# zhvng/open-musiclm

Hardware: AMD Instinct MI355X
Metric: train steps/sec + AR tokens/sec, coarse-stage musiclm_small (higher is better)
Workload: dtype fp16ff; 1 GPU; musiclm_small coarse-stage train step (fwd+bwd+allreduce+clip+AdamW), N=1116 (3 start + 13 clap + 200 semantic + 900 coarse), forgetful mask 0.15, ff_dropout 0.1; global_batch=32, per_gpu_batch=32, grad_accum=1, seq_len=1116, parallelism=dp1, precision=fp16ff, hip_graph=True, exchange=none (single GPU)

## Files before the change

### include/omlm.h

```cpp
#ifndef OMLM_H
#define OMLM_H
#include <stdint.h>
#ifdef __cplusplus
extern "C" {
#endif

int         omlm_version(void);
const char* omlm_last_error(void);
void        omlm_set_error(const char* msg);

int omlm_gemm(const void* A, const void* B, void* C, const float* Cin,
              const int* a_map, const int* b_map, const int* c_map, long long a_rows, long long b_rows,
              int M, int N, int K, int lda, int ldb, int ldc, int ldcin,
              int a_kmajor, int b_kmajor, int in_dtype, int out_dtype, float alpha,
              void* workspace, long long workspace_bytes, void* stream);
long long omlm_gemm_tail_workspace_bytes(int M, int N);

int omlm_layernorm_fwd(const float* x, const float* gamma, void* y, void* xcast, float* mean, float* rstd,
                       int M, int D, int ldy, float eps, int out_dtype, void* stream);
int omlm_layernorm_fwd_planes(const float* x, const float* gamma, void* y, void* y_lo, float* mean, float* rstd,
                              int M, int D, int ldy, float eps, int out_dtype, void* stream);
long long omlm_layernorm_bwd_workspace_bytes(int D);
int omlm_layernorm_bwd2(const void* dy, const float* x, const float* gamma, const float* mean, const float* rstd,
                        const float* dres, const void* dres2, float* dx, void* dxcast, float* dgamma, float* workspace, int M, int D,
                        float dx_scale, int cast_dtype, int dy_dtype, void* stream);

int omlm_qk_norm_fwd(const float* q_raw, const float* kv_raw, const float* q_scale, const float* k_scale,
                     void* q, void* k, void* v, int M, int H, int out_dtype, void* stream);
int omlm_qk_norm_bwd(const float* dq, const float* dk, const float* dv, const float* q_raw, const float* kv_raw,
                     const float* q_scale, const float* k_scale, void* dq_raw, void* dkv_raw,
                     float* dq_scale, float* dk_scale, int M, int H, int out_dtype, void* stream);

int omlm_gemm_qknorm(const void* A, const void* B, void* C, void* C2, int c2_col0, int ldc2, const float* scale, float* norm_out,
                     int ldnorm, int groups, long long a_rows, long long b_rows, int M, int N, int K, int lda, int ldb, int ldc,
                     int dtype, void* stream);
int omlm_qk_norm_bwd2(const float* dq, const float* dk, const float* dv, const void* q, const void* k, const float* qn, const float* kn,
                      const float* q_scale, const float* k_scale, void* dq_raw, void* dkv_raw, float* dq_scale, float* dk_scale,
                      int M, int H, int dtype, void* stream);

int omlm_mqa_attn_fwd(const void* q, const void* k, const void* v, const float* bias, const float* biasT, const unsigned char* keymask,
                      void* out, float* lse, int B, int N, int H, float scale, int bias_ld, int dtype, int P, float p,
                      unsigned long long seed, const unsigned long long* seed_dev, void* stream);
long long omlm_attn_bias_table_floats(int N, int H, int P);
int omlm_attn_bias_prepare(const float* bias, float* biasT, int N, int H, int bias_ld, const float* q_scale,
                           const float* k_scale, float qk_bound, float scale, int p_max_log2, void* stream);
int omlm_attn_bias_prepare_group(const float* bias, float* const* biasT, int layers, int N, int H, int bias_ld,
                                 const float* const* q_scale, const float* const* k_scale, float qk_bound, float scale,
                                 int p_max_log2, int P, void* stream);
long long omlm_mqa_attn_bwd_workspace_bytes(int B, int N, int H);
int omlm_mqa_attn_bwd(const void* q, const void* k, const void* v, const float* bias, const float* biasT, const unsigned char* keymask,
                      const void* out, const void* dout, const float* lse, float* delta, float* dq, float* dk, float* dv, float* dbias,
                      float* dbias_ws, int B, int N, int H, float scale, int bias_ld, int dtype, int P, float p, unsigned long long seed,
                      const unsigned long long* seed_dev, void* stream);
int omlm_attn_dropout_keep(unsigned char* keep, int B, int N, int H, float p, unsigned long long seed,
                           const unsigned long long* seed_dev, void* stream);
int omlm_dropout_residual_fwd(const float* x, const float* y, float* x1, long long M, int D, float p, unsigned long long seed,
                              const unsigned long long* seed_dev, void* stream);
int omlm_dropout_residual_bwd(const float* dx1, void* dy, long long M, int D, float p, unsigned long long seed,
                              const unsigned long long* seed_dev, int out_dtype, void* stream);

int omlm_ffmid_fwd(const void* h1, const void* convw, const void* gamma, void* h2, float* mean, float* rstd,
                   int M, int nseq, int F, int Fp, float eps, float p, unsigned long long seed,
                   const unsigned long long* seed_dev, unsigned char* drop_bits, void* gh, int dtype, void* stream);
int omlm_ffmid_fwd_planes(const void* h1, const void* h1_lo, const void* convw, const void* convw_lo, const void* gamma, const void* gamma_lo,
                          void* h2, void* h2_lo, float* mean, float* rstd, int M, int nseq, int F, int Fp, float eps, float p,
                          unsigned long long seed, const unsigned long long* seed_dev, unsigned char* drop_bits, void* gh, int dtype, void* stream);
long long omlm_ffmid_bwd_workspace_bytes(int F, int Fp);
int omlm_ffmid_bwd(const void* dh2, const void* h1, const void* convw, const void* gamma, const float* mean,
                   const float* rstd, void* du_tmp, void* dh1, float* dgamma, float* dconv, float* workspace,
                   int M, int nseq, int F, int Fp, float p, unsigned long long seed,
                   const unsigned long long* seed_dev, const unsigned char* drop_bits, const void* gh, int dtype, void* stream);
int omlm_colsum_accumulate(const float* part, float* out, int P, int C, int ldp, void* stream);
typedef struct omlm_colsum_desc { const float* part; float* out; int P, C, ldp; } omlm_colsum_desc;
int omlm_colsum_group(const omlm_colsum_desc* problems, int count, void* stream);
int omlm_ffmid_set_impl(int impl);

int omlm_embed_gather_fwd(const int* ids, const int* seg, const int* posidx,
                          const float* const* tables, const float* const* starts, const float* const* pos,
                          int nseq, float* out, int B, int N, int D,
                          const long long* table_rows, const long long* pos_rows, int* err_flag, void* stream);
int omlm_embed_gather_bwd(const int* ids, const int* seg, const int* posidx,
                          float* const* dtables, float* const* dstarts, float* const* dpos,
                          int nseq, const float* dx, int B, int N, int D, float alpha,
                          const long long* table_rows, const long long* pos_rows, int* err_flag, void* stream);

int omlm_prepare_train_batch(const long long* const* ids, int* const* labels, const int* len, const int* eos, const int* Q,
                             const int* codebook, int nseq, int B, int pad_id, const float* scores, int n_drop,
                             int* ids32, unsigned char* keymask, int N, void* stream);

int omlm_cross_entropy_fwd(const float* logits, const int* labels, float* row_lse, float* nll_sum,
                           int R, int V, int ld, int* err_flag, void* stream);
int omlm_cross_entropy_bwd(const float* logits, const int* labels, const float* row_lse, const float* gscale,
                           float coef, void* dlogits, int R, int V, int ld, int ldd, int out_dtype, void* stream);

int omlm_sumsq_accumulate(const float* g, long long n, float* out, float* partials, void* stream);
int omlm_adamw_clip_step(float* p, float* g, float* m, float* v, void* p16, long long n,
                         float lr, float beta1, float beta2, float eps, float wd, int step,
                         float gscale, const float* gnorm_sq, float max_norm, int decoupled, int zero_grad, int p16_dtype,
                         const float* ls_state, void* stream);
int omlm_loss_scale_update(float* ls_state, const float* gnorm_sq, float growth, float backoff, int interval,
                           float scale_min, float scale_max, void* stream);

int omlm_cast_pad(const float* src, void* dst, long long R, int C, int ld_src, int ld_dst, int out_dtype, void* stream);
typedef struct omlm_cast_pad_desc { const float* src; void* dst; int R, C, ld_src, ld_dst, transpose, lo; } omlm_cast_pad_desc;
int omlm_cast_pad_group(const omlm_cast_pad_desc* problems, int count, int out_dtype, void* stream);

int omlm_gemm_planes(const void* A, long long a_plane_bytes, const void* B, long long b_plane_bytes, void* C, const float* Cin,
                     const int* a_map, const int* b_map, const int* c_map, long long a_rows, long long b_rows,
                     int M, int N, int K, int lda, int ldb, int ldc, int ldcin,
                     int a_kmajor, int b_kmajor, int out_dtype, float alpha, void* workspace, long long workspace_bytes, void* stream);
int omlm_split_planes(const float* x, void* planes, long long n, long long plane_elems, void* stream);
int omlm_gemm_planes16(const void* A, const void* A_lo, const void* B, const void* B_lo, void* C, void* C_lo, const float* Cin,
                       const int* a_map, const int* c_map, long long a_rows, long long b_rows, int M, int N, int K,
                       int lda, int ldb, int ldc, int ldcin, int dtype, void* workspace, long long workspace_bytes, void* stream);
int omlm_gemm_mx16(const void* A, const void* A8, long long a8_stride, const unsigned char* a_scale,
                   const void* B, const void* B8, long long b8_stride, const unsigned char* b_scale,
                   void* C, void* C_lo, int c_lo_bf8, const float* Cin, long long a_rows, long long b_rows,
                   int M, int N, int K, int lda, int ldb, int ldc, int ldcin,
                   void* workspace, long long workspace_bytes, void* stream);
long long omlm_gemm_mx16_workspace_bytes(int M, int N, int K);
int omlm_layernorm_fwd_mx(const float* x, const float* gamma, void* y, void* y8, long long y8_stride, unsigned char* scale8,
                          float* mean, float* rstd, int M, int D, int ldy, float eps, void* stream);
int omlm_ffmid_fwd_mx(const void* h1, const void* h1_lo, const void* convw, const void* convw_lo, const void* gamma, const void* gamma_lo,
                      void* h2, void* h2_8, long long h2_8_stride, unsigned char* scale8, float* mean, float* rstd, int M, int nseq, int F, int Fp,
                      float eps, float p, unsigned long long seed, const unsigned long long* seed_dev, unsigned char* drop_bits, void* gh, void* stream);
typedef struct omlm_quant_rows_desc { const float* src; unsigned char* dst8; long long lo_stride; unsigned char* scale8; int R, C, ld_src, ld8; } omlm_quant_rows_desc;
int omlm_quant_rows_mx(const omlm_quant_rows_desc* problems, int count, void* stream);
typedef struct omlm_gemm_wgrad_desc {
    const void* A; const void* B; float* C; const int* c_map;
    int M, N, K, lda, ldb, ldc;
} omlm_gemm_wgrad_desc;
int omlm_gemm_wgrad_group(const omlm_gemm_wgrad_desc* problems, int count, int splits, int dtype, void* stream);

int omlm_relpos_first_fwd(const float* w0, const float* b0, float* pre, float* z, int n, int Hd, int x0, void* stream);
int omlm_relpos_first_bwd(const float* ds, float* dw0, int n, int Hd, int x0, void* stream);
int omlm_bias_silu_fwd(const float* a, const float* b, float* pre, float* z, long long R, int C, void* stream);
int omlm_silu_bwd(const float* dz, const float* pre, float* ds, long long total, void* stream);
int omlm_bias_add(const float* a, const float* b, float* out, int R, int C, int ld, void* stream);
int omlm_relpos_mlp_fwd(const float* w0, const float* b0, const float* W1, const float* b1, const float* W2, const float* b2,
                        const float* W3, const float* b3, float* pre0, float* z0, float* pre1, float* z1, float* pre2, float* z2,
                        float* table, int n, int Hd, int H, int ldb, int x0, void* stream);
int omlm_relpos_mlp_bwd(const float* dtable, const float* W1, const float* W2, const float* W3, const float* pre0, const float* z0,
                        const float* pre1, const float* z1, const float* pre2, const float* z2, float* scratch, float* gw0, float* gb0,
                        float* gW1, float* gb1, float* gW2, float* gb2, float* gW3, float* gb3, int n, int Hd, int H, int ldb, int x0,
                        void* stream);

int omlm_rvq_encode(const float* x, const float* codebooks_T, int* indices, float* residual_out,
                    int n, int D, int C, int nstage, int idx_stride, void* stream);
int omlm_nearest_centroid(const float* x, const float* centroids_T, int* indices, int n, int D, int C, void* stream);
int omlm_vq_accumulate(const float* x, const int* indices, int idx_stride, float* counts, float* sums, int n, int D, int K, void* stream);
int omlm_vq_kmeans_update(float* means, float* means_T, const float* counts, const float* sums, int K, int D, void* stream);
int omlm_vq_ema_update(float* cluster_size, float* embed_avg, float* embed, float* embed_T, const float* counts, const float* sums,
                       float* total_scratch, int K, int D, float decay, float eps, void* stream);

long long omlm_kmeans_pp_workspace_bytes(int m, int trials);
int omlm_kmeans_pp_pick(const float* rows, float* closest, const float* uniforms, int* pick_counter, float* centres, float* centres_T,
                        int* chosen, double* pots, void* workspace, long long workspace_bytes, int m, int D, int K, int trials,
                        void* stream);
int omlm_kmeans_pp_seed(const float* rows, float* closest, const float* uniforms, int* pick_counter, float* centres, float* centres_T,
                        int* chosen, double* pots, void* workspace, long long workspace_bytes, int m, int D, int K, int trials,
                        void* stream);
int omlm_kmeans_minibatch_step(const float* x, const int* idx, float* centres, float* centres_T, float* counts, float* bcounts,
                               float* sums, float* rowmin, double* move_partial, double* state, int n, int B, int D, int K,
                               double alpha, double tol_abs, int max_no_improvement, void* stream);
int omlm_kmeans_inertia(const float* x, const float* centres_T, double* out, int* labels, int n, int D, int K, void* stream);

int omlm_sample_topk_gumbel(const float* logits, const float* uniform, long long* out, int B, int V, int ld,
                            int k, float temperature, int forbid_last, void* stream);

int omlm_sample_topk_gumbel_at(const float* logits, const float* uniform_base, const int* step_dev, long long* out,
                               long long* hist, int B, int V, int ld, int k, float temperature, int forbid_last, void* stream);

int omlm_sample_embed_at(const float* logits, const float* uniform_base, const int* step_dev, long long* out, long long* hist,
                         int B, int V, int ld, int k, float temperature, int forbid_last,
                         const float* emb_table, long long emb_row_offset, long long emb_rows, float* x, int D, void* stream);

typedef struct omlm_decode_args {
    int B, D, H, L, F, Fp, Nmax, w_dtype, round_bf16, nsplit;
    float eps, scale;
    const int* pos_dev;
    const void* const* Wq; const void* const* Wkv; const void* const* Wo; const void* const* W1p; const void* const* W2p;
    const float* const* attn_gamma; const float* const* q_scale; const float* const* k_scale;
    const float* const* ffin_gamma; const float* const* convw; const float* const* mid_gamma;
    float* const* Kc; float* const* Vc; float* const* hist;
    const float* bias_table; int bias_ld;
    const float* final_gamma; const void* head_W; int V1; int ldV;
    const float* emb_table; long long emb_row_offset; long long emb_rows;
    float* x; float* x1; float* q; float* parts; float* u; float* logits;
    int* advance_pos; int* advance_step;
    float* ln_parts;
    const void* const* W1p_lo; const void* const* W2p_lo; const void* head_W_lo;
    float* splitk_ws; int* splitk_cnt;
} omlm_decode_args;
#define OMLM_DECODE_SPLITK_FLOATS(D) (4 * (((D) + 15) / 16) * 256)
#define OMLM_DECODE_LN_PARTS(D, Fp) ((((D) + 15) / 16 > ((Fp) + 7) / 8 ? ((D) + 15) / 16 : ((Fp) + 7) / 8) * 32)
int omlm_decode_step(const omlm_decode_args* args, const long long* ids, void* stream);
int omlm_decode_advance(int* pos_dev, int* step_dev, void* stream);

int omlm_probe_tr16(short* out, void* stream);

#ifdef __cplusplus
}
#endif
#endif
```

### open_musiclm_amd/csrc/ffmid.hip

```cpp
#include "common.h"
#include <stdlib.h>

namespace OMLM_NS {

#define FF_THREADS 256
#define FF_MAXC_LIMIT 16

template <typename T> struct vec8;
template <> struct vec8<float> {
    float v[8];
    __device__ __forceinline__ void load(const float* p) {
        const float4 a = ((const float4*)p)[0], b = ((const float4*)p)[1];
        v[0] = a.x; v[1] = a.y; v[2] = a.z; v[3] = a.w; v[4] = b.x; v[5] = b.y; v[6] = b.z; v[7] = b.w;
    }
    __device__ __forceinline__ void store(float* p) const {
        ((float4*)p)[0] = make_float4(v[0], v[1], v[2], v[3]);
        ((float4*)p)[1] = make_float4(v[4], v[5], v[6], v[7]);
    }
};
template <> struct vec8<h16_t> {
    float v[8];
    __device__ __forceinline__ void load(const h16_t* p) {
        const u32x4 a = *(const u32x4*)p;
#pragma unroll
// ... 374 lines not shown
        }
    }
    __syncthreads();
    for (int c = threadIdx.x; c < Fp; c += FF_THREADS)
        part_dgamma[(size_t)blockIdx.x * Fp + c] = dg_lds[c] + dg_lds[Fp + c] + dg_lds[2 * Fp + c] + dg_lds[3 * Fp + c];
}

template <typename T>
__global__ __launch_bounds__(FF_THREADS) void ffmid_bwd2_kernel(const T* __restrict__ du, const T* __restrict__ h1,
                                                                const T* __restrict__ convw, T* __restrict__ dh1,
                                                                float* __restrict__ part_dconv, int M, int nseq, int F, int Fp) {
    const int ld = 2 * Fp, nchunk = ld / 8;
    const int strips = gridDim.y;
    const int chunk = blockIdx.x * FF_THREADS + threadIdx.x;
    if (chunk >= nchunk) return;
    const int col = chunk * 8;
    const bool gate = col >= Fp;
    const int chreal = gate ? col - Fp : col;
    const int wch = gate ? F + chreal : chreal;
    float w[8][3], dw[8][3];
#pragma unroll
    for (int k = 0; k < 3; ++k) {
        vec8<T> wv;
        wv.load(convw + (size_t)k * ld + col);
#pragma unroll
        for (int i = 0; i < 8; ++i) { w[i][k] = wv.v[i]; dw[i][k] = 0.f; }
    }
    const int rows_per = (M + strips - 1) / strips;
    const int r_begin = blockIdx.y * rows_per, r_end = min(M, r_begin + rows_per);
    vec8<T> da, db, dc, xa, xb, xc;
    zero8(da.v); zero8(db.v); zero8(dc.v); zero8(xa.v); zero8(xb.v); zero8(xc.v);
    if (r_begin < r_end) {
        db.load(du + (size_t)r_begin * ld + col);
        if (r_begin + 1 < M) dc.load(du + (size_t)(r_begin + 1) * ld + col);
        if (r_begin >= 1) xc.load(h1 + (size_t)(r_begin - 1) * ld + col);
        if (r_begin >= 2) xb.load(h1 + (size_t)(r_begin - 2) * ld + col);
    }
    for (int row = r_begin; row < r_end; ++row) {
        const int t = row % nseq;
        da = db; db = dc;
        if (row + 2 < M) dc.load(du + (size_t)(row + 2) * ld + col); else zero8(dc.v);
        xa = xb; xb = xc;
        xc.load(h1 + (size_t)row * ld + col);
        const float m1 = t + 1 < nseq ? 1.f : 0.f, m2 = t + 2 < nseq ? 1.f : 0.f;
        const float p1 = t >= 1 ? 1.f : 0.f, p2 = t >= 2 ? 1.f : 0.f;
        vec8<T> o;
#pragma unroll
        for (int i = 0; i < 8; ++i) {
            o.v[i] = w[i][2] * da.v[i] + w[i][1] * (m1 * db.v[i]) + w[i][0] * (m2 * dc.v[i]);
            dw[i][0] += da.v[i] * (p2 * xa.v[i]);
            dw[i][1] += da.v[i] * (p1 * xb.v[i]);
            dw[i][2] += da.v[i] * xc.v[i];
        }
        o.store(dh1 + (size_t)row * ld + col);
    }
#pragma unroll
    for (int i = 0; i < 8; ++i) {
        if (chreal + i < F) {
#pragma unroll
            for (int k = 0; k < 3; ++k)
                part_dconv[((size_t)blockIdx.y * 2 * F + wch + i) * 3 + k] = dw[i][k];
        }
    }
}

__global__ void colsum_kernel(const float* __restrict__ part, float* __restrict__ out, int P, int C, int ldp) {
    const int c = blockIdx.x * blockDim.x + threadIdx.x;
    if (c >= C) return;
    const int per = (P + gridDim.y - 1) / gridDim.y;
    const int p0 = blockIdx.y * per, p1 = min(P, p0 + per);
    float s = 0.f;
    for (int p = p0; p < p1; ++p) s += part[(size_t)p * ldp + c];
    if (p1 > p0) unsafeAtomicAdd(out + c, s);
}

struct omlm_colsum_desc { const float* part; float* out; int P, C, ldp; };
#define OMLM_COLSUM_MAX 32
struct ColsumGroupArgs { int n; omlm_colsum_desc p[OMLM_COLSUM_MAX]; };
__global__ void colsum_group_kernel(ColsumGroupArgs ga) {
    const omlm_colsum_desc& q = ga.p[blockIdx.z];
    const int c = blockIdx.x * blockDim.x + threadIdx.x;
    if (c >= q.C) return;
    const int per = (q.P + gridDim.y - 1) / gridDim.y;
    const int p0 = blockIdx.y * per, p1 = min(q.P, p0 + per);
    float s = 0.f;
    for (int p = p0; p < p1; ++p) s += q.part[(size_t)p * q.ldp + c];
    if (p1 > p0) unsafeAtomicAdd(q.out + c, s);
}

#if OMLM_FP16
extern "C" int omlm_colsum_accumulate(const float* part, float* out, int P, int C, int ldp, void* stream);
extern "C" int omlm_colsum_group(const omlm_colsum_desc* d, int count, void* stream);
#else
extern "C" int omlm_colsum_group(const omlm_colsum_desc* d, int count, void* stream) {
    if (count <= 0) return OMLM_OK;
    OMLM_CHECK_ARG(d, "colsum_group: null descriptor array");
    for (int base = 0; base < count; base += OMLM_COLSUM_MAX) {
        ColsumGroupArgs ga;
        memset(&ga, 0, sizeof(ga));
        ga.n = count - base < OMLM_COLSUM_MAX ? count - base : OMLM_COLSUM_MAX;
        int cmax = 0, pmax = 0;
        for (int i = 0; i < ga.n; ++i) {
            const omlm_colsum_desc& q = d[base + i];
            OMLM_CHECK_ARG(q.part && q.out && q.P > 0 && q.C > 0 && q.ldp >= q.C, "colsum_group: bad problem");
            ga.p[i] = q;
            if (q.C > cmax) cmax = q.C;
            if (q.P > pmax) pmax = q.P;
        }
        const int ysplit = pmax >= 1024 ? 128 : (pmax >= 64 ? 16 : 1);
        hipLaunchKernelGGL(colsum_group_kernel, dim3((cmax + 255) / 256, ysplit, ga.n), dim3(256), 0, as_stream(stream), ga);
    }
    return omlm_post_launch("omlm_colsum_group");
}

extern "C" int omlm_colsum_accumulate(const float* part, float* out, int P, int C, int ldp, void* stream) {
    if (P <= 0 || C <= 0) return OMLM_OK;
    OMLM_CHECK_ARG(part && out && ldp >= C, "colsum arguments");
    const int ysplit = P >= 1024 ? 128 : (P >= 64 ? 16 : 1);
    hipLaunchKernelGGL(colsum_kernel, dim3((C + 255) / 256, ysplit), dim3(256), 0, as_stream(stream), part, out, P, C, ldp);
    return omlm_post_launch("omlm_colsum_accumulate");
}

#endif

#define FF_BWD1_BLOCKS 1024
#define FF_BWD2_STRIPS 512

bool ffmid2_supported(int Fp);
int ffmid2_fwd_launch(const void* h1, const void* convw, const void* gamma, void* h2, float* mean, float* rstd, int M, int nseq,
                      int F, int Fp, float eps, float p, unsigned long long seed, const unsigned long long* seed_dev,
                      unsigned char* drop_bits, void* gh, int dtype, hipStream_t st);
int ffmid2_bwd_launch(const void* dh2, const void* h1, const void* convw, const void* gamma, const float* rstd, float* bc,
                      void* dh1, float* part_g, int max_g_rows, float* part_c, int max_c_rows, int* g_rows, int* c_rows,
                      int M, int nseq, int F, int Fp, float p, const unsigned char* drop_bits, const void* gh, int dtype, hipStream_t st);
static int g_ffmid_impl = 1;
#if !OMLM_FP16
extern "C" int omlm_ffmid_set_impl_h(int impl);
#endif
extern "C" int OMLM_API(omlm_ffmid_set_impl)(int impl) {
    OMLM_CHECK_ARG(impl == 0 || impl == 1, "impl: 0 = wave-per-row, 1 = column strips");
    g_ffmid_impl = impl;
#if !OMLM_FP16
    return omlm_ffmid_set_impl_h(impl);
#else
    return OMLM_OK;
#endif
}
static int ffmid_impl() { return g_ffmid_impl; }

#if !OMLM_FP16
extern "C" long long omlm_ffmid_bwd_workspace_bytes(int F, int Fp) {
    return (long long)sizeof(float) * ((long long)FF_BWD1_BLOCKS * Fp + (long long)FF_BWD2_STRIPS * 2 * F * 3);
}
#endif

#if !OMLM_FP16
extern "C" int omlm_ffmid_fwd_h(const void* h1, const void* convw, const void* gamma, void* h2, float* mean, float* rstd,
                                int M, int nseq, int F, int Fp, float eps, float p, unsigned long long seed,
                                const unsigned long long* seed_dev, unsigned char* drop_bits, void* gh, int dtype, void* stream);
#endif
extern "C" int OMLM_API(omlm_ffmid_fwd)(const void* h1, const void* convw, const void* gamma, void* h2, float* mean, float* rstd,
                              int M, int nseq, int F, int Fp, float eps, float p, unsigned long long seed,
                              const unsigned long long* seed_dev, unsigned char* drop_bits, void* gh, int dtype, void* stream) {
#if !OMLM_FP16
    if (dtype == OMLM_DT_F16) return omlm_ffmid_fwd_h(h1, convw, gamma, h2, mean, rstd, M, nseq, F, Fp, eps, p, seed, seed_dev, drop_bits, gh, 1, stream);
#else
    OMLM_CHECK_ARG(dtype == 1, "the fp16 copy serves fp16 operands only");
#endif
    if (M <= 0) return OMLM_OK;
    OMLM_CHECK_ARG(h1 && convw && gamma && h2 && mean && rstd, "null pointer");
    OMLM_CHECK_ARG(Fp % 8 == 0 && Fp >= F && Fp <= 8192 && (size_t)5 * Fp * sizeof(float) <= 160 * 1024, "Fp must be F rounded up to 8 and <= 8192");
    OMLM_CHECK_ARG(nseq > 0 && M % nseq == 0, "M must be batch * nseq");
    OMLM_CHECK_ARG(p >= 0.f && p < 1.f, "dropout p");
    hipStream_t st = as_stream(stream);
    if (ffmid_impl() == 1 && ffmid2_supported(Fp) && (p == 0.f || drop_bits))
        return ffmid2_fwd_launch(h1, convw, gamma, h2, mean, rstd, M, nseq, F, Fp, eps, p, seed, seed_dev, drop_bits, gh, dtype, st);
    const int rows4 = (M + 3) / 4;
    dim3 grid(rows4 < 4096 ? rows4 : 4096), block(FF_THREADS);
    const size_t lds_fwd = (size_t)4 * Fp * sizeof(float);
    if (lds_fwd > 48 * 1024) {
#if !OMLM_FP16
        (void)hipFuncSetAttribute((const void*)ffmid_fwd_kernel<float, 8>, hipFuncAttributeMaxDynamicSharedMemorySize, 160 * 1024);
        (void)hipFuncSetAttribute((const void*)ffmid_fwd_kernel<float, 16>, hipFuncAttributeMaxDynamicSharedMemorySize, 160 * 1024);
#endif
        (void)hipFuncSetAttribute((const void*)ffmid_fwd_kernel<h16_t, 8>, hipFuncAttributeMaxDynamicSharedMemorySize, 160 * 1024);
        (void)hipFuncSetAttribute((const void*)ffmid_fwd_kernel<h16_t, 16>, hipFuncAttributeMaxDynamicSharedMemorySize, 160 * 1024);
    }
#define FF_FWD(T_, MC_) hipLaunchKernelGGL((ffmid_fwd_kernel<T_, MC_>), grid, block, lds_fwd, st, (const T_*)h1, (const T_*)convw, (const T_*)gamma, (T_*)h2, mean, rstd, M, nseq, F, Fp, eps, p, seed, seed_dev, drop_bits, (T_*)gh)
#define FF_FWD_DISPATCH(T_) do { const int mc = (Fp / 8 + 63) / 64; \
        if (mc <= 2) FF_FWD(T_, 2); else if (mc <= 6) FF_FWD(T_, 6); else if (mc <= 8) FF_FWD(T_, 8); else FF_FWD(T_, 16); } while (0)
#if !OMLM_FP16
    if (dtype == 0) FF_FWD_DISPATCH(float); else
#endif
    FF_FWD_DISPATCH(h16_t);
    return omlm_post_launch("omlm_ffmid_fwd");
}

int ffmid2_fwd_planes_launch(const void* h1, const void* h1_lo, const void* convw, const void* convw_lo, const void* gamma, const void* gamma_lo,
                             void* h2, void* h2_lo, float* mean, float* rstd, int M, int nseq, int F, int Fp, float eps, float p,
                             unsigned long long seed, const unsigned long long* seed_dev, unsigned char* drop_bits, void* gh, hipStream_t st);
#if !OMLM_FP16
extern "C" int omlm_ffmid_fwd_planes_h(const void* h1, const void* h1_lo, const void* convw, const void* convw_lo, const void* gamma, const void* gamma_lo,
                                       void* h2, void* h2_lo, float* mean, float* rstd, int M, int nseq, int F, int Fp, float eps, float p,
                                       unsigned long long seed, const unsigned long long* seed_dev, unsigned char* drop_bits, void* gh, int dtype, void* stream);
#endif
extern "C" int OMLM_API(omlm_ffmid_fwd_planes)(const void* h1, const void* h1_lo, const void* convw, const void* convw_lo, const void* gamma,
                                               const void* gamma_lo, void* h2, void* h2_lo, float* mean, float* rstd, int M, int nseq, int F, int Fp,
                                               float eps, float p, unsigned long long seed, const unsigned long long* seed_dev,
                                               unsigned char* drop_bits, void* gh, int dtype, void* stream) {
#if !OMLM_FP16
    if (dtype == OMLM_DT_F16)
        return omlm_ffmid_fwd_planes_h(h1, h1_lo, convw, convw_lo, gamma, gamma_lo, h2, h2_lo, mean, rstd, M, nseq, F, Fp, eps, p, seed, seed_dev, drop_bits, gh, 1, stream);
#endif
    OMLM_CHECK_ARG(dtype == 1, "ffmid_fwd_planes: dtype 1 (bf16) or 2 (fp16)");
    if (M <= 0) return OMLM_OK;
    OMLM_CHECK_ARG(h1 && h1_lo && convw && convw_lo && gamma && gamma_lo && h2 && h2_lo && mean && rstd, "null pointer");
    OMLM_CHECK_ARG(Fp % 8 == 0 && Fp >= F && ffmid2_supported(Fp), "ffmid_fwd_planes: Fp must be F rounded up to 8 and <= 4096");
    OMLM_CHECK_ARG(nseq > 0 && M % nseq == 0, "M must be batch * nseq");
    OMLM_CHECK_ARG(p >= 0.f && p < 1.f && (p == 0.f || drop_bits), "dropout p (keep bits required when p > 0)");
    OMLM_CHECK_ARG((((uintptr_t)h1 | (uintptr_t)h1_lo | (uintptr_t)convw | (uintptr_t)convw_lo | (uintptr_t)gamma | (uintptr_t)gamma_lo |
                     (uintptr_t)h2 | (uintptr_t)h2_lo) % 16) == 0, "ffmid_fwd_planes: 16-byte aligned planes");
    return ffmid2_fwd_planes_launch(h1, h1_lo, convw, convw_lo, gamma, gamma_lo, h2, h2_lo, mean, rstd, M, nseq, F, Fp, eps, p, seed, seed_dev,
                                    drop_bits, gh, as_stream(stream));
}

#if OMLM_FP16
int ffmid2_fwd_mx_launch(const void* h1, const void* h1_lo, const void* convw, const void* convw_lo, const void* gamma, const void* gamma_lo,
                         void* h2, void* h2_8, long long h2_8_stride, unsigned char* scale8, float* mean, float* rstd, int M, int nseq, int F, int Fp,
                         float eps, float p, unsigned long long seed, const unsigned long long* seed_dev, unsigned char* drop_bits, void* gh, hipStream_t st);
}
extern "C" int omlm_ffmid_fwd_mx(const void* h1, const void* h1_lo, const void* convw, const void* convw_lo, const void* gamma, const void* gamma_lo,
                                 void* h2, void* h2_8, long long h2_8_stride, unsigned char* scale8, float* mean, float* rstd, int M, int nseq, int F, int Fp,
                                 float eps, float p, unsigned long long seed, const unsigned long long* seed_dev, unsigned char* drop_bits, void* gh,
                                 void* stream) {
    using namespace OMLM_NS;
    if (M <= 0) return OMLM_OK;
    OMLM_CHECK_ARG(h1 && h1_lo && convw && convw_lo && gamma && gamma_lo && h2 && h2_8 && scale8 && mean && rstd, "null pointer");
    OMLM_CHECK_ARG(Fp % 8 == 0 && Fp >= F && ffmid2_supported(Fp), "ffmid_fwd_mx: Fp must be F rounded up to 8 and <= 4096");
    OMLM_CHECK_ARG(nseq > 0 && M % nseq == 0, "M must be batch * nseq");
    OMLM_CHECK_ARG(p >= 0.f && p < 1.f && (p == 0.f || drop_bits), "dropout p (keep bits required when p > 0)");
    OMLM_CHECK_ARG(h2_8_stride >= (long long)M * 2 * Fp && h2_8_stride % 16 == 0, "ffmid_fwd_mx: fp8 plane stride");
    OMLM_CHECK_ARG(2 * Fp >= (Fp + 127) / 128 * 128, "ffmid_fwd_mx: an fp8 plane row (pitch 2 * Fp bytes) must hold Fp rounded up to 128 bytes");
    OMLM_CHECK_ARG((((uintptr_t)h1 | (uintptr_t)h1_lo | (uintptr_t)convw | (uintptr_t)convw_lo | (uintptr_t)gamma | (uintptr_t)gamma_lo |
                     (uintptr_t)h2 | (uintptr_t)h2_8) % 16) == 0, "ffmid_fwd_mx: 16-byte aligned planes");
    return ffmid2_fwd_mx_launch(h1, h1_lo, convw, convw_lo, gamma, gamma_lo, h2, h2_8, h2_8_stride, scale8, mean, rstd, M, nseq, F, Fp, eps, p, seed,
                                seed_dev, drop_bits, gh, as_stream(stream));
}
namespace OMLM_NS {
#endif

#if !OMLM_FP16
extern "C" int omlm_ffmid_bwd_h(const void* dh2, const void* h1, const void* convw, const void* gamma, const float* mean,
                                const float* rstd, void* du_tmp, void* dh1, float* dgamma, float* dconv, float* workspace,
                                int M, int nseq, int F, int Fp, float p, unsigned long long seed,
                                const unsigned long long* seed_dev, const unsigned char* drop_bits, const void* gh, int dtype,
                                void* stream);
#endif
extern "C" int OMLM_API(omlm_ffmid_bwd)(const void* dh2, const void* h1, const void* convw, const void* gamma, const float* mean,
                              const float* rstd, void* du_tmp, void* dh1, float* dgamma, float* dconv, float* workspace,
                              int M, int nseq, int F, int Fp, float p, unsigned long long seed,
                              const unsigned long long* seed_dev, const unsigned char* drop_bits, const void* gh, int dtype,
                              void* stream) {
#if !OMLM_FP16
    if (dtype == OMLM_DT_F16)
        return omlm_ffmid_bwd_h(dh2, h1, convw, gamma, mean, rstd, du_tmp, dh1, dgamma, dconv, workspace, M, nseq, F, Fp, p, seed, seed_dev,
                                drop_bits, gh, 1, stream);
#else
    OMLM_CHECK_ARG(dtype == 1, "the fp16 copy serves fp16 operands only");
#endif
    if (M <= 0) return OMLM_OK;
    OMLM_CHECK_ARG(dh2 && h1 && convw && gamma && mean && rstd && du_tmp && dh1 && workspace, "null pointer");
    OMLM_CHECK_ARG(Fp % 8 == 0 && Fp >= F && Fp <= 8192 && (size_t)5 * Fp * sizeof(float) <= 160 * 1024, "Fp must be F rounded up to 8 and <= 8192");
    OMLM_CHECK_ARG(nseq > 0 && M % nseq == 0, "M must be batch * nseq");
    hipStream_t st = as_stream(stream);
    float* part_g = workspace;
    float* part_c = workspace + (size_t)FF_BWD1_BLOCKS * Fp;
    if (ffmid_impl() == 1 && ffmid2_supported(Fp) && gh && (p == 0.f || drop_bits)) {
        OMLM_CHECK_ARG(((uintptr_t)du_tmp % 8) == 0, "du_tmp must be 8-byte aligned");
        int g_rows = 0, c_rows = 0;
        int rc2 = ffmid2_bwd_launch(dh2, h1, convw, gamma, rstd, (float*)du_tmp, dh1, part_g, FF_BWD1_BLOCKS, part_c, FF_BWD2_STRIPS,
                                    &g_rows, &c_rows, M, nseq, F, Fp, p, drop_bits, gh, dtype, st);
        if (rc2) return rc2;
        if (dgamma && dconv) {
            const omlm_colsum_desc two[2] = {{part_g, dgamma, g_rows, F, Fp}, {part_c, dconv, c_rows, 2 * F * 3, 2 * F * 3}};
            return omlm_colsum_group(two, 2, stream);
        }
        if (dgamma) { rc2 = omlm_colsum_accumulate(part_g, dgamma, g_rows, F, Fp, stream); if (rc2) return rc2; }
        if (dconv)  { rc2 = omlm_colsum_accumulate(part_c, dconv, c_rows, 2 * F * 3, 2 * F * 3, stream); if (rc2) return rc2; }
        return OMLM_OK;
    }
    const int rows4 = (M + 3) / 4;
    const int b1 = rows4 < FF_BWD1_BLOCKS ? rows4 : FF_BWD1_BLOCKS;
    const int strips = M < FF_BWD2_STRIPS ? M : FF_BWD2_STRIPS;
    dim3 g2((2 * Fp / 8 + FF_THREADS - 1) / FF_THREADS, strips);
    const size_t lds1 = (size_t)4 * Fp * sizeof(float);
#define FF_B1_ATTR(T_, MC_) do { (void)hipFuncSetAttribute((const void*)ffmid_bwd1_kernel<T_, MC_, false>, hipFuncAttributeMaxDynamicSharedMemorySize, 160 * 1024); \
        (void)hipFuncSetAttribute((const void*)ffmid_bwd1_kernel<T_, MC_, true>, hipFuncAttributeMaxDynamicSharedMemorySize, 160 * 1024); } while (0)
    if (lds1 > 48 * 1024) {
#if !OMLM_FP16
        FF_B1_ATTR(float, 6); FF_B1_ATTR(float, 8); FF_B1_ATTR(float, 16);
#endif
        FF_B1_ATTR(h16_t, 6); FF_B1_ATTR(h16_t, 8); FF_B1_ATTR(h16_t, 16);
    }
#define FF_B1G(T_, MC_, GH_) hipLaunchKernelGGL((ffmid_bwd1_kernel<T_, MC_, GH_>), dim3(b1), dim3(FF_THREADS), lds1, st, (const T_*)dh2, (const T_*)h1, (const T_*)convw, (const T_*)gamma, mean, rstd, (T_*)du_tmp, part_g, M, nseq, F, Fp, p, seed, seed_dev, drop_bits, (const T_*)gh)
#define FF_B1(T_, MC_) do { if (gh) FF_B1G(T_, MC_, true); else FF_B1G(T_, MC_, false); } while (0)
#define FF_B1_DISPATCH(T_) do { const int mc = (Fp / 8 + 63) / 64; \
// ... 24 lines not shown
```

### open_musiclm_amd/csrc/gemm.hip

```cpp
#include "common.h"
#include "gemm_common.h"

namespace OMLM_NS {

template <int BM_, int BN_, int WM_, int WN_, bool A_KMAJ, bool B_KMAJ, typename TOUT, bool KMAP, bool SPLIT3 = false, bool FASTK = false, int EPI = 0>
__device__ __forceinline__ void gemm_tile_body(const GemmArgs& g, const int lg, const bool split, char* smem) {
    constexpr int NWN = BN_ / WN_, NWAVES = (BM_ / WM_) * NWN;
    constexpr int MI = WM_ / 32, NJ = WN_ / 32;
    constexpr int A_BYTES = BM_ * BK * 2, B_BYTES = BN_ * BK * 2, STAGE = A_BYTES + B_BYTES;
    constexpr int UA = (BM_ / 8) / NWAVES, UB = (BN_ / 8) / NWAVES;

    const int tiles_m = (g.M + BM_ - 1) / BM_, tiles_n = (g.N + BN_ - 1) / BN_;
    const int nwg = tiles_m * tiles_n;
    const int nk1 = (g.K + BK - 1) / BK;
    const int nk_all = SPLIT3 ? 3 * nk1 : nk1;
    constexpr int GROUP = OMLM_SUPER_ROWS / BM_;
    const int lane = threadIdx.x & 63;
    const int wave = __builtin_amdgcn_readfirstlane(threadIdx.x >> 6);
    const int wm = (wave / NWN) * WM_, wn = (wave % NWN) * WN_;
    const dma_rsrc rsA = make_dma_rsrc(g.A, (unsigned long long)g.a_rows * g.lda * 2);
    const dma_rsrc rsB = make_dma_rsrc(g.B, (unsigned long long)g.b_rows * g.ldb * 2);
    const dma_rsrc rsAl = make_dma_rsrc(SPLIT3 ? g.A_lo : g.A, (unsigned long long)g.a_rows * g.lda * 2);
    const dma_rsrc rsBl = make_dma_rsrc(SPLIT3 ? g.B_lo : g.B, (unsigned long long)g.b_rows * g.ldb * 2);

// ... 311 lines not shown
    for (int x = 0; x < 8; ++x)
#pragma unroll
        for (int e = 0; e < 16; ++e) acc[x >> 2][(x >> 1) & 1][x & 1][e] = 0.f;

    auto stage = [&](auto JC, const int T) {
        constexpr int J = decltype(JC)::value;
        constexpr bool isA = (J & 1) != 0;
        constexpr int h = J >> 1;
        const bool live = T < nk;
        unsigned k0 = (unsigned)(kt0 + T) * BK;
        bool lo = false;
        if constexpr (SPLIT3) {
            const int t = kt0 + T, nk1 = g.K / BK;
            const int which = t >= 2 * nk1 ? 2 : (t >= nk1 ? 1 : 0);
            k0 = (unsigned)(t - which * nk1) * BK;
            lo = isA ? which == 2 : which == 1;
        }
        const dma_rsrc rs = isA ? (SPLIT3 && lo ? rsAl : rsA) : (SPLIT3 && lo ? rsBl : rsB);
        if constexpr (SPLIT3) k0 = (unsigned)__builtin_amdgcn_readfirstlane((int)k0);
        const unsigned base = smem_lds + (unsigned)((T & 1) * STAGE) + (isA ? 0u : (unsigned)A_BYTES);
#pragma unroll
        for (int u = 0; u < 2; ++u) {
            const int i = 2 * h + u;
            const int b = wave + 8 * i;
            if constexpr (isA) dma_issue_s(rs, base + (unsigned)(b * 1024), live ? sa.vfast[i] : OOB_OFF, A_KMAJ ? k0 * (unsigned)(g.lda * 2) : k0 * 2u);
            else               dma_issue_s(rs, base + (unsigned)(b * 1024), live ? sb.vfast[i] : OOB_OFF, B_KMAJ ? k0 * (unsigned)(g.ldb * 2) : k0 * 2u);
        }
    };
    using J0 = std::integral_constant<int, 0>; using J1 = std::integral_constant<int, 1>;
    using J2 = std::integral_constant<int, 2>; using J3 = std::integral_constant<int, 3>;

    h16x8 a[2][4], bX[4], bY[4], bZ[4];
    auto read_a = [&](const int T, const int ha) {
        const char* As = smem + (T & 1) * STAGE;
#pragma unroll
        for (int i = 0; i < 2; ++i)
#pragma unroll
            for (int st = 0; st < 4; ++st) a[i][st] = read_frag<A_KMAJ>(As, ha * 128 + wr * 64 + 32 * i, st, lane);
    };
    auto read_b = [&](h16x8 (&b)[4], const int T, const int hb) {
        const char* Bs = smem + (T & 1) * STAGE + A_BYTES;
#pragma unroll
        for (int st = 0; st < 4; ++st) b[st] = read_frag<B_KMAJ>(Bs, hb * 128 + wc * 32, st, lane);
    };
    auto mma = [&](f32x16 (&c)[2], const h16x8 (&b)[4]) {
        __builtin_amdgcn_s_setprio(1);
#pragma unroll
        for (int st = 0; st < 4; ++st)
#pragma unroll
            for (int i = 0; i < 2; ++i) c[i] = OMLM_MFMA_32x32x16(a[i][st], b[st], c[i]);
        __builtin_amdgcn_s_setprio(0);
    };
#define T8_SYNC_IN()                                                           \
    do {                                                                       \
        __builtin_amdgcn_sched_barrier(0);                                     \
        asm volatile("s_waitcnt vmcnt(10)" ::: "memory");                      \
        __builtin_amdgcn_s_barrier();                                          \
        asm volatile("s_waitcnt lgkmcnt(0)" ::: "memory");                     \
        __builtin_amdgcn_sched_barrier(0);                                     \
    } while (0)
#define T8_SYNC_OUT()                                                          \
    do {                                                                       \
        __builtin_amdgcn_sched_barrier(0);                                     \
        __builtin_amdgcn_s_barrier();                                          \
        __builtin_amdgcn_sched_barrier(0);                                     \
    } while (0)

    stage(J0{}, 0); stage(J1{}, 0); stage(J2{}, 0); stage(J3{}, 0);
    stage(J0{}, 1); stage(J1{}, 1); stage(J2{}, 1);
    asm volatile("s_waitcnt vmcnt(10)" ::: "memory");
    __builtin_amdgcn_s_barrier();
    read_b(bX, 0, 0);
    asm volatile("s_waitcnt lgkmcnt(0)" ::: "memory");
    __builtin_amdgcn_sched_barrier(0);
    if (wr == 1) __builtin_amdgcn_s_barrier();

    auto ktile = [&](h16x8 (&b0)[4], h16x8 (&bn)[4], const int T) {
        read_a(T, 0);             stage(J3{}, T + 1);  T8_SYNC_IN();  mma(acc[0][0], b0);  T8_SYNC_OUT();
        read_b(bY, T, 1);         stage(J0{}, T + 2);  T8_SYNC_IN();  mma(acc[0][1], bY);  T8_SYNC_OUT();
        read_a(T, 1);             stage(J1{}, T + 2);  T8_SYNC_IN();  mma(acc[1][1], bY);  T8_SYNC_OUT();
        read_b(bn, T + 1, 0);     stage(J2{}, T + 2);  T8_SYNC_IN();  mma(acc[1][0], b0);  T8_SYNC_OUT();
    };
    for (int T = 0; T < nk; T += 2) {
        ktile(bX, bZ, T);
        if (T + 1 < nk) ktile(bZ, bX, T + 1);
    }
    if (wr == 0) __builtin_amdgcn_s_barrier();
#undef T8_SYNC_IN
#undef T8_SYNC_OUT
    asm volatile("s_waitcnt vmcnt(0)" ::: "memory");
    __syncthreads();
#pragma unroll
    for (int ha = 0; ha < 2; ++ha)
#pragma unroll
        for (int hb = 0; hb < 2; ++hb)
            tile_epilogue<2, 1, 32, TOUT>(g, reinterpret_cast<f32x16 (&)[2][1]>(acc[ha][hb]), smem, m0, n0, ha * 128 + wr * 64, hb * 128 + wc * 32,
                                          wave, lane, split);
}

template <bool A_KMAJ, bool B_KMAJ, typename TOUT, bool SPLIT3 = false>
__global__ __launch_bounds__(512) void gemm_tile8_kernel(GemmArgs g) {
    extern __shared__ __attribute__((aligned(16))) char smem[];
    const int nwg = gridDim.x;
    const int lg = xcd_logical_id(blockIdx.y * nwg + blockIdx.x, nwg * (int)gridDim.y);
    const int tiles_m = (g.M + 255) / 256, tiles_n = (g.N + 255) / 256;
    const int ksplit = lg / nwg, bid = lg - ksplit * nwg;
    const int nk_all = (SPLIT3 ? 3 : 1) * (g.K / BK);
    const int kt0 = ksplit * g.kt_per_split, kt1 = min(nk_all, kt0 + g.kt_per_split);
    constexpr int GROUP = OMLM_SUPER_ROWS / 256;
    const int gsz = GROUP * tiles_n;
    const int grp = bid / gsz, first_m = grp * GROUP;
    const int rows_in = min(GROUP, tiles_m - first_m);
    const int tm = first_m + (bid - grp * gsz) % rows_in, tn = (bid - grp * gsz) / rows_in;
    if (kt0 >= kt1) return;
    gemm_tile8_body<A_KMAJ, B_KMAJ, TOUT, SPLIT3>(g, tm * 256, tn * 256, kt0, kt1, gridDim.y > 1, smem);
}


#define OMLM_GROUP_MAX 48
struct omlm_gemm_wgrad_desc { const void* A; const void* B; float* C; const int* c_map; int M, N, K, lda, ldb, ldc; };
struct GroupProb { const void* A; const void* B; float* C; const int* c_map; int M, N, K, lda, ldb, ldc, kt_per_split, start; };
struct GroupArgs { int n, total; GroupProb p[OMLM_GROUP_MAX]; };

template <bool FASTK, bool T8 = false>
__global__ __launch_bounds__(512) void gemm_wgrad_group_kernel(GroupArgs ga) {
    extern __shared__ __attribute__((aligned(16))) char smem[];
    const int lg = xcd_logical_id(blockIdx.x, ga.total);
    int pi = 0;
    for (int i = 1; i < ga.n; ++i) if (lg >= ga.p[i].start) pi = i;
    const GroupProb& q = ga.p[pi];
    GemmArgs g;
    g.A = q.A; g.B = q.B; g.C = q.C; g.Cin = q.C; g.a_map = nullptr; g.b_map = nullptr; g.c_map = q.c_map;
    g.a_rows = q.K; g.b_rows = q.K; g.M = q.M; g.N = q.N; g.K = q.K; g.lda = q.lda; g.ldb = q.ldb; g.ldc = q.ldc; g.ldcin = q.ldc;
    g.alpha = 1.f; g.kt_per_split = q.kt_per_split; g.bal_ck = 0; g.bal_chunks = 0; g.debug = 0; g.split3 = 0; g.A_lo = nullptr; g.B_lo = nullptr; g.C_lo = nullptr; g.c_lo8 = 0; g.c_split_stride = 0;
    g.epi_scale = nullptr; g.epi_norm = nullptr; g.epi_groups = 0; g.epi_ldnorm = 0; g.C2 = nullptr; g.c2_col0 = 0; g.ldc2 = 0;
    const int nk = (q.K + BK - 1) / BK;
    if constexpr (T8) {
        const int lq = lg - q.start;
        const int tiles_m = (q.M + 255) / 256, tiles_n = (q.N + 255) / 256, nwg = tiles_m * tiles_n;
        const int ksplit = lq / nwg, bid = lq - ksplit * nwg;
        const int kt0 = ksplit * q.kt_per_split, kt1 = min(nk, kt0 + q.kt_per_split);
        constexpr int GROUP = OMLM_SUPER_ROWS / 256;
        const int gsz = GROUP * tiles_n;
        const int grp = bid / gsz, first_m = grp * GROUP;
        const int rows_in = min(GROUP, tiles_m - first_m);
        const int tm = first_m + (bid - grp * gsz) % rows_in, tn = (bid - grp * gsz) / rows_in;
        if (kt0 < kt1) gemm_tile8_body<true, true, float>(g, tm * 256, tn * 256, kt0, kt1, q.kt_per_split < nk, smem);
    } else {
        gemm_tile_body<256, 256, 128, 64, true, true, float, false, false, FASTK>(g, lg - q.start, q.kt_per_split < nk, smem);
    }
}


#ifdef OMLM_ISA_ONLY
template __global__ void gemm_bf16_tile_persist_kernel<256, 256, 128, 64, false, false, h16_t, false>(GemmArgs);
template __global__ void gemm_bf16_tile_persist_kernel<256, 256, 128, 64, false, true, h16_t, false>(GemmArgs);
template __global__ void gemm_bf16_tile_persist_kernel<256, 256, 128, 64, false, false, float, true>(GemmArgs);
template __global__ void gemm_bf16_tile_persist_kernel<256, 256, 128, 64, false, true, float, true>(GemmArgs);
template __global__ void gemm_bf16_tile_persist_kernel<128, 128, 64, 64, false, false, h16_t, false>(GemmArgs);
template __global__ void gemm_bf16_tile_persist_kernel<128, 128, 64, 64, false, false, float, true>(GemmArgs);
template __global__ void gemm_bf16_tile_persist_kernel<128, 128, 64, 64, false, false, h16_t, false, 1>(GemmArgs);
template __global__ void gemm_tile8_kernel<false, false, h16_t>(GemmArgs);
template __global__ void gemm_tile8_kernel<false, true, h16_t>(GemmArgs);
template __global__ void gemm_tile8_kernel<false, false, float>(GemmArgs);
template __global__ void gemm_tile8_kernel<true, true, float>(GemmArgs);
template __global__ void gemm_tile8_kernel<false, false, h16pl_t, true>(GemmArgs);
template __global__ void gemm_tile8_kernel<false, false, float, true>(GemmArgs);
}
#else
static int gemm_persist_slots() {
    static int ncu8 = -1;
    if (ncu8 < 0) {
        int dev = 0, n = 0;
        ncu8 = (hipGetDevice(&dev) == hipSuccess && hipDeviceGetAttribute(&n, hipDeviceAttributeMultiprocessorCount, dev) == hipSuccess && n >= 8) ? n / 8 * 8 : 0;
    }
    const char* e = getenv("OMLM_GEMM_PERSIST");
    return (e && e[0] == '0') ? 0 : ncu8;
}

static int gemm_t8_mode() {
    const char* e = getenv("OMLM_GEMM_T8");
    return e ? atoi(e) : OMLM_GEMM_T8_DEFAULT;
}
static bool gemm_t8_wanted(int K, int tiles, int splits) {
    const int mode = gemm_t8_mode();
    if (mode <= 0) return false;
    if (mode == 1) return true;
    static int ncu = 0;
    if (ncu == 0) {
        int dev = 0, n = 0;
        ncu = (hipGetDevice(&dev) == hipSuccess && hipDeviceGetAttribute(&n, hipDeviceAttributeMultiprocessorCount, dev) == hipSuccess && n > 0) ? n : 256;
    }
    return splits == 1 && K >= 2048 && tiles > ncu;
}

template <int BM_, int BN_, int WM_, int WN_, typename TOUT>
static int launch_tile(const GemmArgs& g, int a_kmaj, int b_kmaj, int splits, hipStream_t st) {
    constexpr int NTH = (BM_ / WM_) * (BN_ / WN_) * 64;
    constexpr size_t LDS = 2 * (size_t)(BM_ + BN_) * BK * 2;
    const int tiles = ((g.M + BM_ - 1) / BM_) * ((g.N + BN_ - 1) / BN_);
    dim3 grid(tiles, splits), block(NTH);
    if constexpr (BM_ == 256 && BN_ == 256) {
        if (gemm_t8_wanted(g.split3 ? 3 * g.K : g.K, tiles, splits) && g.K % BK == 0 && !g.a_map && !g.b_map &&
            (!g.split3 || !OMLM_FP16)) {
#define OMLM_T8_LAUNCH(AK, BKM)                                                                                       \
            do {                                                                                                       \
                auto k8 = gemm_tile8_kernel<AK, BKM, TOUT>;                                                            \
                static bool attr8 = false;                                                                             \
                if (!attr8) { (void)hipFuncSetAttribute((const void*)k8, hipFuncAttributeMaxDynamicSharedMemorySize, (int)LDS); attr8 = true; } \
                if constexpr (!OMLM_FP16) {                                                                            \
                    auto k83 = gemm_tile8_kernel<AK, BKM, TOUT, true>;                                                 \
                    static bool attr83 = false;                                                                        \
                    if (!attr83) { (void)hipFuncSetAttribute((const void*)k83, hipFuncAttributeMaxDynamicSharedMemorySize, (int)LDS); attr83 = true; } \
                    if (g.split3) { hipLaunchKernelGGL(k83, grid, block, LDS, st, g); break; }                         \
                }                                                                                                      \
                hipLaunchKernelGGL(k8, grid, block, LDS, st, g);                                                       \
            } while (0)
            if (!a_kmaj && !b_kmaj)      OMLM_T8_LAUNCH(false, false);
            else if (!a_kmaj && b_kmaj)  OMLM_T8_LAUNCH(false, true);
            else if (a_kmaj && b_kmaj)   OMLM_T8_LAUNCH(true, true);
            else                         OMLM_T8_LAUNCH(true, false);
#undef OMLM_T8_LAUNCH
            return omlm_post_launch("omlm_gemm");
        }
    }
    const bool need_kmap = (a_kmaj && g.a_map) || (b_kmaj && g.b_map);
    if (need_kmap && BM_ != 128) { omlm_set_error("omlm_gemm: k-row maps are only built for the 128x128 tile"); return OMLM_ERR_UNSUPPORTED; }
#define OMLM_TILE_LAUNCH(AK, BKM)                                                                                          \
    do {                                                                                                                    \
        auto kfn = gemm_bf16_tile_kernel<BM_, BN_, WM_, WN_, AK, BKM, TOUT, false>;                                        \
        auto kmap = gemm_bf16_tile_kernel<BM_, BN_, WM_, WN_, AK, BKM, TOUT, (AK || BKM) && BM_ == 128>;                   \
        auto kfast = gemm_bf16_tile_kernel<BM_, BN_, WM_, WN_, AK, BKM, TOUT, false, false, true>;                         \
        static bool attr = false;                                                                                           \
        if (!attr) {                                                                                                        \
            (void)hipFuncSetAttribute((const void*)kfn, hipFuncAttributeMaxDynamicSharedMemorySize, (int)LDS);             \
            (void)hipFuncSetAttribute((const void*)kfast, hipFuncAttributeMaxDynamicSharedMemorySize, (int)LDS);           \
            (void)hipFuncSetAttribute((const void*)kmap, hipFuncAttributeMaxDynamicSharedMemorySize, (int)LDS);            \
        }                                                                                                                   \
        if constexpr (!OMLM_FP16) {                                                                                         \
            auto ks3 = gemm_bf16_tile_kernel<BM_, BN_, WM_, WN_, AK, BKM, TOUT, false, true>;                               \
            if (!attr) (void)hipFuncSetAttribute((const void*)ks3, hipFuncAttributeMaxDynamicSharedMemorySize, (int)LDS);  \
            attr = true;                                                                                                    \
            if (g.split3) { hipLaunchKernelGGL(ks3, grid, block, LDS, st, g); break; }                                     \
        }                                                                                                                   \
        attr = true;                                                                                                        \
        if (need_kmap) hipLaunchKernelGGL(kmap, grid, block, LDS, st, g);                                                  \
        else if (g.K % BK == 0) hipLaunchKernelGGL(kfast, grid, block, LDS, st, g);                                        \
        else           hipLaunchKernelGGL(kfn, grid, block, LDS, st, g);                                                   \
    } while (0)
    if constexpr ((BM_ == 256 && BN_ == 256) || (BM_ == 128 && BN_ == 128)) {
        const int slots = gemm_persist_slots() * (BM_ == 128 ? 2 : 1);
        if (slots > 0 && !a_kmaj && splits == 1 && !g.split3 && !g.a_map && !g.b_map && !g.c_map && g.K % BK == 0 && tiles > slots) {
            constexpr size_t LDSP = LDS + 32 * (WN_ + 4) * 4;
            static bool pattr = false;
            auto k0 = gemm_bf16_tile_persist_kernel<BM_, BN_, WM_, WN_, false, false, TOUT, false>;
            auto k1 = gemm_bf16_tile_persist_kernel<BM_, BN_, WM_, WN_, false, true, TOUT, false>;
            auto k0c = gemm_bf16_tile_persist_kernel<BM_, BN_, WM_, WN_, false, false, TOUT, true>;
            auto k1c = gemm_bf16_tile_persist_kernel<BM_, BN_, WM_, WN_, false, true, TOUT, true>;
            if (!pattr) {
                (void)hipFuncSetAttribute((const void*)k0, hipFuncAttributeMaxDynamicSharedMemorySize, (int)LDSP);
                (void)hipFuncSetAttribute((const void*)k1, hipFuncAttributeMaxDynamicSharedMemorySize, (int)LDSP);
                (void)hipFuncSetAttribute((const void*)k0c, hipFuncAttributeMaxDynamicSharedMemorySize, (int)LDSP);
                (void)hipFuncSetAttribute((const void*)k1c, hipFuncAttributeMaxDynamicSharedMemorySize, (int)LDSP);
                pattr = true;
            }
            hipLaunchKernelGGL(g.Cin ? (b_kmaj ? k1c : k0c) : (b_kmaj ? k1 : k0), dim3(slots), block, LDSP, st, g);
            return omlm_post_launch("omlm_gemm");
        }
    }
    if (!a_kmaj && !b_kmaj)      OMLM_TILE_LAUNCH(false, false);
    else if (!a_kmaj && b_kmaj)  OMLM_TILE_LAUNCH(false, true);
    else if (a_kmaj && b_kmaj)   OMLM_TILE_LAUNCH(true, true);
    else                         OMLM_TILE_LAUNCH(true, false);
#undef OMLM_TILE_LAUNCH
    return omlm_post_launch("omlm_gemm");
}

template <int BM_, int BN_, int WM_, int WN_, typename TOUT>
static int launch_tile_s3(const GemmArgs& g, hipStream_t st, int splits = 1) {
    constexpr int NTH = (BM_ / WM_) * (BN_ / WN_) * 64;
    constexpr size_t LDS = 2 * (size_t)(BM_ + BN_) * BK * 2;
    const int tiles = ((g.M + BM_ - 1) / BM_) * ((g.N + BN_ - 1) / BN_);
    dim3 grid(tiles, splits), block(NTH);
    if constexpr (BM_ == 256 && BN_ == 256) {
        if (gemm_t8_mode() > 0 && g.K % BK == 0 && !g.a_map && splits == 1) {
            auto k8 = gemm_tile8_kernel<false, false, TOUT, true>;
            static bool attr8 = false;
            if (!attr8) { (void)hipFuncSetAttribute((const void*)k8, hipFuncAttributeMaxDynamicSharedMemorySize, (int)LDS); attr8 = true; }
            hipLaunchKernelGGL(k8, grid, block, LDS, st, g);
            return omlm_post_launch("omlm_gemm_planes16");
        }
    }
    auto ks3 = gemm_bf16_tile_kernel<BM_, BN_, WM_, WN_, false, false, TOUT, false, true>;
    static bool attr = false;
    if (!attr) { (void)hipFuncSetAttribute((const void*)ks3, hipFuncAttributeMaxDynamicSharedMemorySize, (int)LDS); attr = true; }
    hipLaunchKernelGGL(ks3, grid, block, LDS, st, g);
    return omlm_post_launch("omlm_gemm_planes16");
}

template <typename T, typename TOUT>
static int launch_layout(const GemmArgs& g, int a_kmaj, int b_kmaj, int splits, hipStream_t st) {
    const int tiles = ((g.M + BM - 1) / BM) * ((g.N + BN - 1) / BN);
    const size_t lds = 4 * (size_t)(BM * BK * 2);
    dim3 grid(tiles, splits), block(NTHREADS);
    if constexpr (elt_traits<T>::precise) {
        if (!a_kmaj && !b_kmaj)      hipLaunchKernelGGL((gemm_kernel<T, false, false, TOUT>), grid, block, lds, st, g);
        else if (!a_kmaj && b_kmaj)  hipLaunchKernelGGL((gemm_kernel<T, false, true, TOUT>), grid, block, lds, st, g);
// ... 92 lines not shown
        if (s3_route) {
            if (tm_ == 256 && tn_ == 256)
                return ga.C_lo ? launch_tile_s3<256, 256, 128, 64, h16pl_t>(ga, st) : launch_tile_s3<256, 256, 128, 64, float>(ga, st);
            if (tm_ == 256 && tn_ == 128)
                return ga.C_lo ? launch_tile_s3<256, 128, 64, 64, h16pl_t>(ga, st) : launch_tile_s3<256, 128, 64, 64, float>(ga, st);
            return ga.C_lo ? launch_tile_s3<128, 128, 64, 64, h16pl_t>(ga, st) : launch_tile_s3<128, 128, 64, 64, float>(ga, st);
        }
        if (tm_ == 256 && tn_ == 256)
            return out_dtype == 0 ? launch_tile<256, 256, 128, 64, float>(ga, a_kmajor, b_kmajor, sp, st)
                                  : launch_tile<256, 256, 128, 64, h16_t>(ga, a_kmajor, b_kmajor, sp, st);
        if (tm_ == 256 && tn_ == 128)
            return out_dtype == 0 ? launch_tile<256, 128, 64, 64, float>(ga, a_kmajor, b_kmajor, sp, st)
                                  : launch_tile<256, 128, 64, 64, h16_t>(ga, a_kmajor, b_kmajor, sp, st);
        return out_dtype == 0 ? launch_tile<128, 128, 64, 64, float>(ga, a_kmajor, b_kmajor, sp, st)
                              : launch_tile<128, 128, 64, 64, h16_t>(ga, a_kmajor, b_kmajor, sp, st);
    };
    if (bm == 256 && bn == 256 && splits == 1 && !a_kmajor && !a_map && !c_map && !(force && force[0]) && tiles > ncu) {
        const int tiles_n = (N + 255) / 256, tiles_m = (M + 255) / 256;
        const int rem = tiles % ncu;
        const int m_full = ((tiles / ncu) * ncu) / tiles_n;
        if (rem > 0 && rem < ncu / 2 && m_full >= 1 && m_full < tiles_m) {
            const size_t osz = out_dtype == 0 ? 4 : 2;
            const long long M1 = (long long)m_full * 256;
            GemmArgs g1 = g, g2 = g;
            g1.M = (int)M1;
            g2.M = M - (int)M1;
            g2.A = (const char*)A + (size_t)M1 * lda * 2;
            g2.a_rows = a_rows - M1;
            g2.C = (char*)C + (size_t)M1 * ldc * osz;
            if (g.A_lo && !a_kmajor) g2.A_lo = (const char*)g.A_lo + (size_t)M1 * lda * 2;
            if (g.C_lo) g2.C_lo = (char*)g.C_lo + (size_t)M1 * ldc * osz;
            if (Cin) g2.Cin = Cin + (size_t)M1 * ldcin;
            const int rc = launch(g1, 256, 256, 1);
            if (rc != OMLM_OK) return rc;
            if (tail_ws && gemm_tail_split_on() && alpha == 1.0f) {
                const int Mt = g2.M, Nw = (N + 3) / 4 * 4;
                const int tiles_t = ((Mt + 127) / 128) * ((N + 127) / 128);
                int S = (2 * ncu) / tiles_t;
                if (S > nk / 8) S = nk / 8;
                if (S > 8) S = 8;
                if (S >= 2) {
                    const int ktps = (nk + S - 1) / S;
                    S = (nk + ktps - 1) / ktps;
                    const long long slice = (long long)Mt * Nw;
                    if (S >= 2 && (long long)S * slice * 4 <= tail_ws_bytes) {
                        GemmArgs gw = g2;
                        gw.C = tail_ws; gw.C_lo = nullptr; gw.Cin = nullptr; gw.ldc = Nw; gw.ldcin = 0;
                        gw.c_split_stride = slice; gw.kt_per_split = ktps;
                        const int rc2 = s3_route ? launch_tile_s3<128, 128, 64, 64, float>(gw, st, S)
                                                 : launch_tile<128, 128, 64, 64, float>(gw, a_kmajor, b_kmajor, S, st);
                        if (rc2 != OMLM_OK) return rc2;
                        const long long quads = (long long)Mt * (Nw / 4);
                        const int blocks = (int)((quads + 255) / 256 > 4096 ? 4096 : (quads + 255) / 256);
                        if (out_dtype == 0)
                            hipLaunchKernelGGL(gemm_tail_reduce_kernel<0>, dim3(blocks), dim3(256), 0, st, tail_ws, S, slice, Mt, N, Nw, g2.C, nullptr, ldc, g2.Cin, ldcin);
                        else if (g2.C_lo)
                            hipLaunchKernelGGL(gemm_tail_reduce_kernel<2>, dim3(blocks), dim3(256), 0, st, tail_ws, S, slice, Mt, N, Nw, g2.C, g2.C_lo, ldc, g2.Cin, ldcin);
                        else
                            hipLaunchKernelGGL(gemm_tail_reduce_kernel<1>, dim3(blocks), dim3(256), 0, st, tail_ws, S, slice, Mt, N, Nw, g2.C, nullptr, ldc, g2.Cin, ldcin);
                        return omlm_post_launch("omlm_gemm (tail reduce)");
                    }
                }
            }
            return launch(g2, 128, 128, 1);
        }
    }
    return launch(g, bm, bn, splits);
}

#if !OMLM_FP16
extern "C" long long omlm_gemm_tail_workspace_bytes(int M, int N) {
    if (M <= 0 || N <= 0) return 0;
    int dev = 0, ncu = 256;
    if (hipGetDevice(&dev) == hipSuccess) (void)hipDeviceGetAttribute(&ncu, hipDeviceAttributeMultiprocessorCount, dev);
    const long long tiles_n = (N + 255) / 256, tiles_m = (M + 255) / 256;
    if (tiles_m * tiles_n <= ncu) return 0;
    long long tail_rows = ((long long)(ncu / 2) / tiles_n + 1) * 256;
    if (tail_rows > M) tail_rows = M;
    return 8ll * tail_rows * ((N + 3) / 4 * 4) * 4;
}
#endif

#if !OMLM_FP16
extern "C" int omlm_gemm_h(const void* A, const void* B, void* C, const float* Cin, const int* a_map, const int* b_map, const int* c_map,
                           long long a_rows, long long b_rows, int M, int N, int K, int lda, int ldb, int ldc, int ldcin,
                           int a_kmajor, int b_kmajor, int in_dtype, int out_dtype, float alpha, void* workspace, long long workspace_bytes, void* stream);
#endif
extern "C" int OMLM_API(omlm_gemm)(const void* A, const void* B, void* C, const float* Cin,
                         const int* a_map, const int* b_map, const int* c_map,
                         long long a_rows, long long b_rows,
                         int M, int N, int K, int lda, int ldb, int ldc, int ldcin,
                         int a_kmajor, int b_kmajor, int in_dtype, int out_dtype, float alpha, void* workspace, long long workspace_bytes, void* stream) {
#if !OMLM_FP16
    if (in_dtype == OMLM_DT_F16) {
        OMLM_CHECK_ARG(out_dtype == OMLM_DT_F32 || out_dtype == OMLM_DT_F16, "fp16 operands produce fp32 or fp16 output");
        return omlm_gemm_h(A, B, C, Cin, a_map, b_map, c_map, a_rows, b_rows, M, N, K, lda, ldb, ldc, ldcin, a_kmajor, b_kmajor,
                           1, OMLM_H_CODE(out_dtype), alpha, workspace, workspace_bytes, stream);
    }
#endif
    OMLM_CHECK_ARG((workspace == nullptr) == (workspace_bytes == 0) && workspace_bytes >= 0 && ((uintptr_t)workspace % 16) == 0,
                   "tail workspace: 16-byte aligned buffer and its size, or NULL / 0");
    return gemm_impl(A, B, C, Cin, a_map, b_map, c_map, a_rows, b_rows, M, N, K, lda, ldb, ldc, ldcin, a_kmajor, b_kmajor,
                     in_dtype, out_dtype, alpha, stream, 0, nullptr, nullptr, nullptr, false, (float*)workspace, workspace_bytes);
}

#if !OMLM_FP16
extern "C" int omlm_gemm_qknorm_h(const void* A, const void* B, void* C, void* C2, int c2_col0, int ldc2, const float* scale, float* norm_out,
                                  int ldnorm, int groups, long long a_rows, long long b_rows, int M, int N, int K, int lda, int ldb, int ldc,
                                  int dtype, void* stream);
#endif
extern "C" int OMLM_API(omlm_gemm_qknorm)(const void* A, const void* B, void* C, void* C2, int c2_col0, int ldc2, const float* scale,
                                          float* norm_out, int ldnorm, int groups, long long a_rows, long long b_rows, int M, int N, int K,
                                          int lda, int ldb, int ldc, int dtype, void* stream) {
#if !OMLM_FP16
    if (dtype == OMLM_DT_F16) return omlm_gemm_qknorm_h(A, B, C, C2, c2_col0, ldc2, scale, norm_out, ldnorm, groups, a_rows, b_rows, M, N, K, lda, ldb, ldc, 1, stream);
#endif
    if (M <= 0 || N <= 0) return OMLM_OK;
    OMLM_CHECK_ARG(dtype == 1, "gemm_qknorm: operand dtype 1 (bf16) or 2 (fp16)");
    OMLM_CHECK_ARG(A && B && C && scale && norm_out && K > 0 && (K % 8) == 0, "gemm_qknorm: null operand / K");
    OMLM_CHECK_ARG((N % 64) == 0 && groups >= 0 && groups * 64 <= N && ldnorm >= groups, "gemm_qknorm: N must be whole 64-wide heads");
    OMLM_CHECK_ARG((lda % 8) == 0 && (ldb % 8) == 0 && (ldc % 8) == 0 && ((uintptr_t)A % 16) == 0 && ((uintptr_t)B % 16) == 0 && ((uintptr_t)C % 16) == 0,
                   "gemm_qknorm: 16-byte aligned operands, pitches multiples of 8");
    OMLM_CHECK_ARG(!C2 || ((c2_col0 % 64) == 0 && (ldc2 % 8) == 0 && ((uintptr_t)C2 % 16) == 0), "gemm_qknorm: second output");
    OMLM_CHECK_ARG((unsigned long long)a_rows * lda * 2 < 0xFFFFFFF0ull && (unsigned long long)b_rows * ldb * 2 < 0xFFFFFFF0ull, "operand exceeds the 4 GiB window");
    GemmArgs g;
    memset(&g, 0, sizeof(g));
    g.A = A; g.B = B; g.C = C; g.a_rows = a_rows; g.b_rows = b_rows; g.M = M; g.N = N; g.K = K; g.lda = lda; g.ldb = ldb; g.ldc = ldc;
    g.alpha = 1.f; g.epi_scale = scale; g.epi_norm = norm_out; g.epi_groups = groups; g.epi_ldnorm = ldnorm; g.C2 = C2; g.c2_col0 = c2_col0; g.ldc2 = ldc2;
    const int nk = (K + BK - 1) / BK;
    g.kt_per_split = nk;
    constexpr size_t LDS = 2 * (size_t)(128 + 128) * BK * 2;
    const int tiles = ((M + 127) / 128) * ((N + 127) / 128);
    auto kfast = gemm_bf16_tile_kernel<128, 128, 64, 64, false, false, h16_t, false, false, true, 1>;
    auto kgen = gemm_bf16_tile_kernel<128, 128, 64, 64, false, false, h16_t, false, false, false, 1>;
    static bool attr = false;
    if (!attr) {
        (void)hipFuncSetAttribute((const void*)kfast, hipFuncAttributeMaxDynamicSharedMemorySize, (int)LDS);
        (void)hipFuncSetAttribute((const void*)kgen, hipFuncAttributeMaxDynamicSharedMemorySize, (int)LDS);
        attr = true;
    }
    const int slots = 2 * gemm_persist_slots();
    if (slots > 0 && tiles > slots && K % BK == 0) {
        constexpr size_t LDSP = LDS + 32 * (64 + 4) * 4;
        auto kp = gemm_bf16_tile_persist_kernel<128, 128, 64, 64, false, false, h16_t, false, 1>;
        static bool pattr = false;
        if (!pattr) { (void)hipFuncSetAttribute((const void*)kp, hipFuncAttributeMaxDynamicSharedMemorySize, (int)LDSP); pattr = true; }
        hipLaunchKernelGGL(kp, dim3(slots), dim3(256), LDSP, as_stream(stream), g);
    }
    else if (K % BK == 0) hipLaunchKernelGGL(kfast, dim3(tiles, 1), dim3(256), LDS, as_stream(stream), g);
    else                                        hipLaunchKernelGGL(kgen, dim3(tiles, 1), dim3(256), LDS, as_stream(stream), g);
    return omlm_post_launch("omlm_gemm_qknorm");
}

#if !OMLM_FP16
extern "C" int omlm_gemm_planes16_h(const void* A, const void* A_lo, const void* B, const void* B_lo, void* C, void* C_lo, const float* Cin,
                                    const int* a_map, const int* c_map, long long a_rows, long long b_rows, int M, int N, int K,
                                    int lda, int ldb, int ldc, int ldcin, int dtype, void* workspace, long long workspace_bytes, void* stream);
#endif
extern "C" int OMLM_API(omlm_gemm_planes16)(const void* A, const void* A_lo, const void* B, const void* B_lo, void* C, void* C_lo, const float* Cin,
                                            const int* a_map, const int* c_map, long long a_rows, long long b_rows, int M, int N, int K,
                                            int lda, int ldb, int ldc, int ldcin, int dtype, void* workspace, long long workspace_bytes, void* stream) {
#if !OMLM_FP16
    if (dtype == OMLM_DT_F16) return omlm_gemm_planes16_h(A, A_lo, B, B_lo, C, C_lo, Cin, a_map, c_map, a_rows, b_rows, M, N, K, lda, ldb, ldc, ldcin, 1,
                                                          workspace, workspace_bytes, stream);
#endif
    OMLM_CHECK_ARG((workspace == nullptr) == (workspace_bytes == 0) && workspace_bytes >= 0 && ((uintptr_t)workspace % 16) == 0,
                   "tail workspace: 16-byte aligned buffer and its size, or NULL / 0");
    OMLM_CHECK_ARG(dtype == 1, "gemm_planes16: operand dtype 1 (bf16) or 2 (fp16)");
    OMLM_CHECK_ARG(A_lo && B_lo, "gemm_planes16: null lo plane");
    OMLM_CHECK_ARG(((uintptr_t)A_lo % 16) == 0 && ((uintptr_t)B_lo % 16) == 0 && ((uintptr_t)C_lo % 16) == 0, "gemm_planes16: 16-byte aligned planes");
    OMLM_CHECK_ARG(!(C_lo && Cin), "gemm_planes16: plane output takes no residual");
    return gemm_impl(A, B, C, Cin, a_map, nullptr, c_map, a_rows, b_rows, M, N, K, lda, ldb, ldc, ldcin, 0, 0,
                     1, C_lo ? 1 : 0, 1.0f, stream, 1, A_lo, B_lo, C_lo, true, (float*)workspace, workspace_bytes);
}

#if !OMLM_FP16
extern "C" int omlm_gemm_planes(const void* A, long long a_plane_bytes, const void* B, long long b_plane_bytes, void* C, const float* Cin,
                                const int* a_map, const int* b_map, const int* c_map, long long a_rows, long long b_rows,
                                int M, int N, int K, int lda, int ldb, int ldc, int ldcin,
                                int a_kmajor, int b_kmajor, int out_dtype, float alpha, void* workspace, long long workspace_bytes, void* stream) {
    OMLM_CHECK_ARG((workspace == nullptr) == (workspace_bytes == 0) && workspace_bytes >= 0 && ((uintptr_t)workspace % 16) == 0,
                   "tail workspace: 16-byte aligned buffer and its size, or NULL / 0");
    OMLM_CHECK_ARG(a_plane_bytes > 0 && b_plane_bytes > 0 && (a_plane_bytes % 16) == 0 && (b_plane_bytes % 16) == 0, "plane strides");
    OMLM_CHECK_ARG(!(a_kmajor && a_map) && !(b_kmajor && b_map), "k-row maps are not supported on operand planes");
    return gemm_impl(A, B, C, Cin, a_map, b_map, c_map, a_rows, b_rows, M, N, K, lda, ldb, ldc, ldcin, a_kmajor, b_kmajor,
                     1, out_dtype, alpha, stream, 1, (const char*)A + a_plane_bytes, (const char*)B + b_plane_bytes, nullptr, false,
                     (float*)workspace, workspace_bytes);
}

__global__ __launch_bounds__(256) void split_planes_kernel(const float* __restrict__ x, unsigned short* __restrict__ planes,
                                                           long long n, long long plane_elems) {
    const long long i0 = ((long long)blockIdx.x * 256 + threadIdx.x) * 8;
    const long long stride = (long long)gridDim.x * 256 * 8;
    for (long long i = i0; i < n; i += stride) {
        if (i + 8 <= n) {
            const float4 a = *(const float4*)(x + i), b = *(const float4*)(x + i + 4);
            unsigned h0, h1, h2, h3, l0, l1, l2, l3;
            split_pair(a.x, a.y, h0, l0); split_pair(a.z, a.w, h1, l1);
            split_pair(b.x, b.y, h2, l2); split_pair(b.z, b.w, h3, l3);
            u32x4 hi, lo;
            hi[0] = h0; hi[1] = h1; hi[2] = h2; hi[3] = h3; lo[0] = l0; lo[1] = l1; lo[2] = l2; lo[3] = l3;
            *(u32x4*)(planes + i) = hi;
            *(u32x4*)(planes + plane_elems + i) = lo;
        } else {
            for (long long j = i; j < n; ++j) {
                const unsigned u = f2u(x[j]) & 0xFFFF0000u;
                planes[j] = (unsigned short)(u >> 16);
                planes[plane_elems + j] = (unsigned short)bf16_bits_rne(x[j] - u2f(u));
            }
        }
    }
}
extern "C" int omlm_split_planes(const float* x, void* planes, long long n, long long plane_elems, void* stream) {
    if (n <= 0) return OMLM_OK;
    OMLM_CHECK_ARG(x && planes && plane_elems >= n && (plane_elems % 8) == 0, "split_planes arguments");
    OMLM_CHECK_ARG(((uintptr_t)x % 16) == 0 && ((uintptr_t)planes % 16) == 0, "split_planes: 16-byte aligned buffers");
    long long blocks = (n / 8 + 255) / 256;
    if (blocks > 16384) blocks = 16384;
    if (blocks < 1) blocks = 1;
    hipLaunchKernelGGL(split_planes_kernel, dim3((unsigned)blocks), dim3(256), 0, as_stream(stream), x, (unsigned short*)planes, n, plane_elems);
    return omlm_post_launch("omlm_split_planes");
}

#endif

#if !OMLM_FP16
extern "C" int omlm_gemm_wgrad_group_h(const omlm_gemm_wgrad_desc* d, int count, int splits, int dtype, void* stream);
#endif
extern "C" int OMLM_API(omlm_gemm_wgrad_group)(const omlm_gemm_wgrad_desc* d, int count, int splits, int dtype, void* stream) {
    if (count <= 0) return OMLM_OK;
    OMLM_CHECK_ARG(d, "null descriptor array");
#if !OMLM_FP16
    if (dtype == OMLM_DT_F16) return omlm_gemm_wgrad_group_h(d, count, splits, 1, stream);
#endif
    OMLM_CHECK_ARG(dtype == 1, "wgrad group: operand dtype must be 1 (bf16) or 2 (fp16)");
    static int ncu = 0;
    if (ncu == 0) {
        int dev = 0, n = 0;
        if (hipGetDevice(&dev) == hipSuccess && hipDeviceGetAttribute(&n, hipDeviceAttributeMultiprocessorCount, dev) == hipSuccess && n > 0) ncu = n;
        else ncu = 256;
    }
    static bool attr = false;
    if (!attr) {
        (void)hipFuncSetAttribute((const void*)gemm_wgrad_group_kernel<false>, hipFuncAttributeMaxDynamicSharedMemorySize, 131072);
        (void)hipFuncSetAttribute((const void*)gemm_wgrad_group_kernel<true>, hipFuncAttributeMaxDynamicSharedMemorySize, 131072);
        (void)hipFuncSetAttribute((const void*)gemm_wgrad_group_kernel<true, true>, hipFuncAttributeMaxDynamicSharedMemorySize, 131072);
        attr = true;
    }
    for (int base = 0; base < count; base += OMLM_GROUP_MAX) {
        const int n = count - base < OMLM_GROUP_MAX ? count - base : OMLM_GROUP_MAX;
        long long units = 0;
        int nk_min = 1 << 30;
        bool fastk = true;
        for (int i = 0; i < n; ++i) {
            const omlm_gemm_wgrad_desc& q = d[base + i];
            if (q.K % BK != 0) fastk = false;
            OMLM_CHECK_ARG(q.A && q.B && q.C && q.M > 0 && q.N > 0 && q.K > 0, "wgrad group: bad problem");
            OMLM_CHECK_ARG((q.lda % 8) == 0 && (q.ldb % 8) == 0 && q.lda >= ((q.M + 7) / 8) * 8 && q.ldb >= ((q.N + 7) / 8) * 8,
                           "wgrad group: k-major operand pitches must be multiples of 8 covering the padded extent");
            OMLM_CHECK_ARG(((uintptr_t)q.A % 16) == 0 && ((uintptr_t)q.B % 16) == 0, "wgrad group: operands must be 16-byte aligned");
            OMLM_CHECK_ARG((unsigned long long)q.K * q.lda * 2 < 0xFFFFFFF0ull && (unsigned long long)q.K * q.ldb * 2 < 0xFFFFFFF0ull,
                           "wgrad group: operand exceeds the 4 GiB buffer-descriptor window");
            units += (long long)((q.M + 255) / 256) * ((q.N + 255) / 256);
            const int nk = (q.K + BK - 1) / BK;
            if (nk < nk_min) nk_min = nk;
        }
        int sp = splits;
        if (sp <= 0) {
            float best = -1.f;
            sp = 1;
            for (int s = 1; s <= 4; ++s) {
                const long long wgs = units * s, rounds = (wgs + ncu - 1) / ncu;
                const float util = (float)wgs / (float)(rounds * ncu) - 0.02f * (float)(s - 1);
                if (util > best) { best = util; sp = s; }
            }
        }
        if (sp > nk_min / 8) sp = nk_min / 8 > 0 ? nk_min / 8 : 1;
        GroupArgs ga;
        memset(&ga, 0, sizeof(ga));
        ga.n = n;
        int start = 0;
        for (int i = 0; i < n; ++i) {
            const omlm_gemm_wgrad_desc& q = d[base + i];
            GroupProb& p = ga.p[i];
            p.A = q.A; p.B = q.B; p.C = q.C; p.c_map = q.c_map; p.M = q.M; p.N = q.N; p.K = q.K; p.lda = q.lda; p.ldb = q.ldb; p.ldc = q.ldc;
            const int nk = (q.K + BK - 1) / BK;
            p.kt_per_split = (nk + sp - 1) / sp;
            const int s_eff = (nk + p.kt_per_split - 1) / p.kt_per_split;
            p.start = start;
            start += ((q.M + 255) / 256) * ((q.N + 255) / 256) * s_eff;
        }
        ga.total = start;
        if (fastk && gemm_t8_mode() > 0) hipLaunchKernelGGL((gemm_wgrad_group_kernel<true, true>), dim3(start), dim3(512), 131072, as_stream(stream), ga);
        else if (fastk) hipLaunchKernelGGL(gemm_wgrad_group_kernel<true>, dim3(start), dim3(512), 131072, as_stream(stream), ga);
        else       hipLaunchKernelGGL(gemm_wgrad_group_kernel<false>, dim3(start), dim3(512), 131072, as_stream(stream), ga);
    }
    return omlm_post_launch("omlm_gemm_wgrad_group");
}

}
#endif
```

### open_musiclm_amd/engine.py

```python
from __future__ import annotations

import math
import os
from dataclasses import dataclass, field
from typing import Dict, List, Optional, Sequence, Tuple

import torch

from . import ops
from .hip import require_gpu

ATTN_SCALE = 8.0
DIM_HEAD = 64

_PRECISIONS = {"bf16": torch.bfloat16, "bf16x3": torch.float32, "fp16": torch.float16, "fp16ff": torch.float16}


def is_half(precision: str) -> bool:
    return precision in ("fp16", "fp16ff")
_H16 = (torch.bfloat16, torch.float16)



FF_PLANES_MAX_FP = 4096
# ... 296 lines not shown
    dev = tr.norm.gamma.device
    rows, x0 = relpos_rows(n, P)
    if tr.relative_position_bias_type == "t5":
        from .transformer import t5_bucket_of_distance
        bucket = t5_bucket_of_distance(torch.arange(x0, n, device=dev), rp.num_buckets, rp.max_distance)
        table = torch.zeros(rows, ldb, device=dev, dtype=torch.float32)
        table[:, :H] = rp.relative_attention_bias.weight.detach()[bucket]
        return table, ("t5", bucket)
    lin = [rp.net[0][0], rp.net[1][0], rp.net[2][0], rp.net[3]]
    Hd = lin[0].weight.shape[0]
    if Hd in (256, 512) and H <= 16 and len(rp.net) == 4:
        saves = [torch.empty(rows, Hd, device=dev) for _ in range(6)] if save else None
        table = torch.empty(rows, ldb, device=dev)
        ops.relpos_mlp_fwd(lin[0].weight.detach().reshape(-1), lin[0].bias.detach(), lin[1].weight.detach(), lin[1].bias.detach(),
                           lin[2].weight.detach(), lin[2].bias.detach(), lin[3].weight.detach(), lin[3].bias.detach(), saves, table, rows, Hd, H, ldb,
                           x0=x0)
        return table, (("mlp_fused", saves) if save else None)
    n = rows
    pres, zs = [], []
    pre = torch.empty(n, Hd, device=dev)
    z = torch.empty(n, Hd, device=dev)
    ops.relpos_first_fwd(lin[0].weight.detach().reshape(-1), lin[0].bias.detach(), pre, z, n, Hd, x0=x0)
    pres.append(pre); zs.append(z)
    for k in (1, 2):
        a = torch.empty(n, Hd, device=dev)
        ops.gemm(zs[-1], lin[k].weight.detach(), a, M=n, N=Hd, K=Hd, planes=False)
        pre = torch.empty(n, Hd, device=dev)
        z = torch.empty(n, Hd, device=dev)
        ops.bias_silu_fwd(a, lin[k].bias.detach(), pre, z, n, Hd)
        pres.append(pre); zs.append(z)
    a = torch.zeros(n, ldb, device=dev)
    ops.gemm(zs[-1], lin[3].weight.detach(), a, M=n, N=H, K=Hd, ldc=ldb)
    table = torch.empty(n, ldb, device=dev)
    ops.bias_add(a, lin[3].bias.detach(), table, n, H, ldb)
    return table, (("mlp", pres, zs) if save else None)


def relpos_backward(tr, n: int, saved, dtable: torch.Tensor):
    rp = tr.rel_pos_bias
    H = tr.heads
    ldb = dtable.shape[-1]
    dev = dtable.device
    x0 = n - dtable.shape[0]
    n = dtable.shape[0]
    if saved[0] == "t5":
        g = grad_of(rp.relative_attention_bias.weight)
        g.index_add_(0, saved[1], dtable[:, :H])
        return
    lin = [rp.net[0][0], rp.net[1][0], rp.net[2][0], rp.net[3]]
    Hd = lin[0].weight.shape[0]
    if saved[0] == "mlp_fused":
        scratch = torch.empty(3 * n * Hd, device=dev)
        grads = [grad_of(lin[0].weight).view(-1), grad_of(lin[0].bias), grad_of(lin[1].weight), grad_of(lin[1].bias),
                 grad_of(lin[2].weight), grad_of(lin[2].bias), grad_of(lin[3].weight), grad_of(lin[3].bias)]
        ops.relpos_mlp_bwd(dtable, lin[1].weight.detach(), lin[2].weight.detach(), lin[3].weight.detach(), saved[1], scratch, grads, n, Hd, H, ldb,
                           x0=x0)
        return
    _, pres, zs = saved
    ops.colsum_accumulate(dtable, grad_of(lin[3].bias), n, H, ldb)
    gw = grad_of(lin[3].weight)
    ops.gemm(dtable, zs[2], gw, M=H, N=Hd, K=n, a_kmajor=True, b_kmajor=True, Cin=gw, lda=ldb)
    dz = torch.empty(n, Hd, device=dev)
    ops.gemm(dtable, lin[3].weight.detach(), dz, M=n, N=Hd, K=ldb, b_kmajor=True, lda=ldb, b_rows=H)
    for k in (2, 1):
        ds = torch.empty(n, Hd, device=dev)
        ops.silu_bwd(dz, pres[k], ds, n * Hd)
        ops.colsum_accumulate(ds, grad_of(lin[k].bias), n, Hd, Hd)
        gw = grad_of(lin[k].weight)
        ops.gemm(ds, zs[k - 1], gw, M=Hd, N=Hd, K=n, a_kmajor=True, b_kmajor=True, Cin=gw, planes=False)
        dz = torch.zeros(n, Hd, device=dev)
        ops.gemm(ds, lin[k].weight.detach(), dz, M=n, N=Hd, K=Hd, b_kmajor=True, Cin=dz, planes=False)
    ds = torch.empty(n, Hd, device=dev)
    ops.silu_bwd(dz, pres[0], ds, n * Hd)
    ops.colsum_accumulate(ds, grad_of(lin[0].bias), n, Hd, Hd)
    ops.relpos_first_bwd(ds, grad_of(lin[0].weight).view(-1), n, Hd, x0=x0)


class LayerSaved:
    __slots__ = ("x", "m1", "r1", "xn", "xc", "q_raw", "kv_raw", "q", "k", "v", "o", "lse", "abias",
                 "x1", "m2", "r2", "xn2", "h1", "h2", "m3", "r3", "seed", "p", "drop_bits", "gh", "h1_lo_tail",
                 "pa", "sa", "po", "so")


def _dropout_state(tr, dev):
    st = tr.__dict__.get("_omlm_dropout")
    if st is None or st["counter"].device != dev:
        rank = int(os.environ.get("RANK", "0"))
        g = torch.Generator().manual_seed((int(torch.initial_seed()) + 0x9E3779B1 * rank) & 0x7FFFFFFF)
        L = len(tr.layers)
        st = dict(counter=torch.zeros(1, dtype=torch.int64, device=dev),
                  seeds=[int(v) for v in torch.randint(1, 2 ** 62, (L,), generator=g)])
        a = [int(v) for v in torch.randint(1, 2 ** 62, (2 * L,), generator=g)]
        st["attn_seeds"], st["out_seeds"] = a[:L], a[L:]
        st["last"] = None
        tr.__dict__["_omlm_dropout"] = st
    return st


def dropout_salt(tr, dev) -> torch.Tensor:
    st = _dropout_state(tr, dev)
    st["counter"].add_(1)
    st["last"] = st["counter"].clone()
    return st["last"], st["seeds"]


def dropout_state(tr, dev=None) -> dict:
    st = tr.__dict__.get("_omlm_dropout")
    if st is None:
        st = _dropout_state(tr, dev if dev is not None else torch.device("cpu"))
    last = st["last"]
    return dict(ff=list(st["seeds"]), attn=list(st["attn_seeds"]), out=list(st["out_seeds"]),
                salt=int(last.item()) if last is not None else None)


def trunk_forward(tr, pw: PreparedWeights, x: torch.Tensor, keymask: Optional[torch.Tensor], B: int, N: int,
                  save: bool, training: bool, keep_h1_lo_tail: bool = False):
    T = pw.T
    dev = x.device
    M, D = x.shape
    H = tr.heads
    P = prefix_rows(tr)
    rc = tr.__dict__.get("_omlm_relpos_cache")
    if rc is not None and save and training and rc.usable(N):
        table, rp_saved = rc.table, ("cached", rc)
    else:
        table, rp_saved = relpos_forward(tr, N, save, P)
        if (rc is not None and rc.enabled and rc.n is None and save and training and rp_saved is not None and rp_saved[0] != "t5"
                and not torch.cuda.is_current_stream_capturing()):
            rc.adopt(N, table, rp_saved)
            rp_saved = ("cached", rc)
    saved_layers: List[LayerSaved] = []
    abiases = None
    salt, seeds, aseeds, oseeds = (None, None, None, None)
    aps = [(float(a_.attn_dropout.p), float(a_.to_out[1].p)) if training else (0.0, 0.0) for a_, _, _ in tr.layers]
    if training and (any(float(ff.dropout_p) > 0 for _, _, ff in tr.layers) or any(pa > 0 or po > 0 for pa, po in aps)):
        salt, seeds = dropout_salt(tr, dev)
        st_ = tr.__dict__["_omlm_dropout"]
        aseeds, oseeds = st_["attn_seeds"], st_["out_seeds"]
    for li, ((attn, _, ff), w) in enumerate(zip(tr.layers, pw.layers)):
        sv = LayerSaved()
        F, Fp = w["F"], w["Fp"]
        m1 = torch.empty(M, device=dev); r1 = torch.empty(M, device=dev)
        xn = torch.empty(M, D, dtype=T, device=dev)
        xc = x if T == torch.float32 else torch.empty(M, D, dtype=T, device=dev)
        ops.layernorm_fwd(x, attn.norm.gamma.detach(), xn, None if T == torch.float32 else xc, m1, r1)
        q = torch.empty(M, H * DIM_HEAD, dtype=T, device=dev)
        k = torch.empty(M, DIM_HEAD, dtype=T, device=dev)
        v = torch.empty(M, DIM_HEAD, dtype=T, device=dev)
        fused_qk = T in _H16
        if fused_qk:
            qn = torch.empty(M, H, device=dev)
            kn = torch.empty(M, device=dev)
            q_raw, kv_raw = qn, kn
            ops.gemm_qknorm(xn, w["Wq"], q, attn.q_scale.detach(), qn, H, M=M, N=H * DIM_HEAD, K=D)
            ops.gemm_qknorm(xc, w["Wkv"], k, attn.k_scale.detach(), kn, 1, M=M, N=2 * DIM_HEAD, K=D, C2=v, c2_col0=DIM_HEAD)
        else:
            q_raw = torch.empty(M, H * DIM_HEAD, device=dev)
            kv_raw = torch.empty(M, 2 * DIM_HEAD, device=dev)
            ops.gemm(xn, w["Wq"], q_raw, M=M, N=H * DIM_HEAD, K=D)
            ops.gemm(xc, w["Wkv"], kv_raw, M=M, N=2 * DIM_HEAD, K=D)
            ops.qk_norm_fwd(q_raw, kv_raw, attn.q_scale.detach(), attn.k_scale.detach(), q, k, v, H)
        o = torch.empty(M, H * DIM_HEAD, dtype=T, device=dev)
        lse = torch.empty(B, H, N, device=dev)
        if abiases is None:
            abiases = ops.AttnBias.group(table, N, H, dev, [a_.q_scale.detach() for a_, _, _ in tr.layers],
                                         [a_.k_scale.detach() for a_, _, _ in tr.layers], scale=ATTN_SCALE, half=T == torch.float16, P=P)
        abias = abiases[li]
        pa, po = aps[li]
        sa = aseeds[li] if pa > 0 else 0
        so = oseeds[li] if po > 0 else 0
        ops.attn_fwd(q, k, v, abias, keymask, o, lse, B, N, H, ATTN_SCALE, P=P, p=pa, seed=sa, seed_dev=salt if pa > 0 else None)
        x1 = torch.empty(M, D, device=dev)
        if po > 0:
            yo = torch.empty(M, D, device=dev)
            ops.gemm(o, w["Wo"], yo, M=M, N=D, K=H * DIM_HEAD)
            ops.dropout_residual_fwd(x, yo, x1, po, so, seed_dev=salt)
            del yo
        else:
            ops.gemm(o, w["Wo"], x1, M=M, N=D, K=H * DIM_HEAD, Cin=x)
        m2 = torch.empty(M, device=dev); r2 = torch.empty(M, device=dev)
        xn2 = torch.empty(M, D, dtype=T, device=dev)
        h1 = torch.empty(M, 2 * Fp, dtype=T, device=dev)
        if pw.mx:
            P1 = ops.Fp8Planes(M, D, dev, zero=False)
            ops.layernorm_fwd_mx(x1, ff.norm_in.gamma.detach(), xn2, P1, m2, r2)
            h1_lo = torch.empty(M, 2 * Fp, dtype=torch.uint8, device=dev)
            ops.gemm_mx16(xn2, P1, w["W1p"], w["W1p8"], h1, h1_lo, M=M, N=2 * Fp, K=D)
        elif pw.ff_planes:
            xn2_lo = torch.empty(M, D, dtype=T, device=dev)
            ops.layernorm_fwd_planes(x1, ff.norm_in.gamma.detach(), xn2, xn2_lo, m2, r2)
            h1_lo = torch.empty(M, 2 * Fp, dtype=T, device=dev)
            ops.gemm_planes16(xn2, xn2_lo, w["W1p"], w["W1p_lo"], h1, h1_lo, M=M, N=2 * Fp, K=D)
        else:
            ops.layernorm_fwd(x1, ff.norm_in.gamma.detach(), xn2, None, m2, r2)
            ops.gemm(xn2, w["W1p"], h1, M=M, N=2 * Fp, K=D)
        h2 = torch.empty(M, Fp, dtype=T, device=dev)
        m3 = torch.empty(M, device=dev); r3 = torch.empty(M, device=dev)
        p = float(ff.dropout_p) if training else 0.0
        seed = seeds[li] if (p > 0 and seeds is not None) else 0
        drop_bits = torch.empty(M, Fp // 8, dtype=torch.uint8, device=dev) if (p > 0 and (save or pw.ff_planes)) else None
        gh = torch.empty(M, Fp, dtype=T, device=dev) if save else None
        x2 = torch.empty(M, D, device=dev)
        if pw.ff_planes:
            if pw.mx:
                P2 = ops.Fp8Planes(M, Fp, dev, zero=False)
                ops.ffmid_fwd_mx(h1, h1_lo, w["convw"], w["convw_lo"], w["gamma_mid"], w["gamma_mid_lo"], h2, P2, m3, r3, N, F, Fp, p, seed,
                                 seed_dev=salt if p > 0 else None, drop_bits=drop_bits, gh=gh)
                ops.gemm_mx16(h2, P2, w["W2p"], w["W2p8"], x2, M=M, N=D, K=Fp, Cin=x1)
            else:
                h2_lo = torch.empty(M, Fp, dtype=T, device=dev)
                ops.ffmid_fwd_planes(h1, h1_lo, w["convw"], w["convw_lo"], w["gamma_mid"], w["gamma_mid_lo"], h2, h2_lo, m3, r3, N, F, Fp, p, seed,
                                     seed_dev=salt if p > 0 else None, drop_bits=drop_bits, gh=gh)
                ops.gemm_planes16(h2, h2_lo, w["W2p"], w["W2p_lo"], x2, M=M, N=D, K=Fp, Cin=x1)
                del xn2_lo, h2_lo
            if keep_h1_lo_tail and save:
                take = min(2, N)
                sv.h1_lo_tail = torch.zeros(B, 2, 2 * Fp, device=dev)
                tail = h1_lo.view(B, N, -1)[:, N - take:]
                if tail.dtype == torch.uint8:
                    tail = (tail.contiguous().to(torch.int16) << 8).view(torch.float16)
                sv.h1_lo_tail[:, 2 - take:].copy_(tail)
            del h1_lo
        else:
            ops.ffmid_fwd(h1, w["convw"], w["gamma_mid"], h2, m3, r3, N, F, Fp, p, seed, seed_dev=salt if p > 0 else None,
                          drop_bits=drop_bits, gh=gh)
            ops.gemm(h2, w["W2p"], x2, M=M, N=D, K=Fp, Cin=x1)
        if save:
            sv.x, sv.m1, sv.r1, sv.xn, sv.xc = x, m1, r1, xn, xc
            sv.q_raw, sv.kv_raw, sv.q, sv.k, sv.v, sv.o, sv.lse, sv.abias = q_raw, kv_raw, q, k, v, o, lse, abias
            sv.x1, sv.m2, sv.r2, sv.xn2, sv.h1, sv.h2, sv.m3, sv.r3, sv.seed, sv.p = x1, m2, r2, xn2, h1, h2, m3, r3, seed, p
            sv.drop_bits = drop_bits
            sv.gh = gh
            sv.pa, sv.sa, sv.po, sv.so = pa, sa, po, so
            saved_layers.append(sv)
        x = x2
    mf = torch.empty(M, device=dev); rf = torch.empty(M, device=dev)
    y, y_lo = torch.empty(M, D, dtype=T, device=dev), None
    if pw.ff3:
        y_lo = torch.empty(M, D, dtype=T, device=dev)
        ops.layernorm_fwd_planes(x, tr.norm.gamma.detach(), y, y_lo, mf, rf)
    else:
        ops.layernorm_fwd(x, tr.norm.gamma.detach(), y, None, mf, rf)
    saved = dict(layers=saved_layers, xL=x, mf=mf, rf=rf, table=table, rp=rp_saved, keymask=keymask, salt=salt) if save else None
    return y, y_lo, saved


def trunk_backward(tr, pw: PreparedWeights, saved, dy: torch.Tensor, B: int, N: int, out_scale: float, head_wgrads=None):
    T = pw.T
    dev = dy.device
    M, D = dy.shape
    H = tr.heads
    table, keymask = saved["table"], saved["keymask"]
    rp_cached = saved["rp"] is not None and saved["rp"][0] == "cached"
    dtable = (saved["rp"][1].dtable if rp_cached else torch.zeros_like(table)) if table is not None else None
    nl = len(saved["layers"])
    dres = torch.empty(M, D, device=dev)
    dres_c = dres if T == torch.float32 else torch.empty(M, D, dtype=T, device=dev)
    cg = ops.ColsumGroup()
    ops.layernorm_bwd(dy, saved["xL"], tr.norm.gamma.detach(), saved["mf"], saved["rf"], None, dres,
                      None if T == torch.float32 else dres_c, grad_of(tr.norm.gamma),
                      dx_scale=out_scale if nl == 0 else 1.0, defer=cg)
    ws = None
    wg = ops.WgradGroup() if T in _H16 else None
    for dYh, Xh, dWh, Mo, No in (head_wgrads or []):
        if wg is not None:
            wg.add(dYh, Xh, dWh, M=Mo, N=No, K=dYh.shape[0])
        else:
            ops.gemm(dYh, Xh, dWh, M=Mo, N=No, K=dYh.shape[0], a_kmajor=True, b_kmajor=True, Cin=dWh)

    def wgrad(dY, X, dW, Mo, No, c_map=None):
        if wg is not None:
            wg.add(dY, X, dW, M=Mo, N=No, K=M, c_map=c_map)
            if len(wg.items) >= 40:
                wg.flush()
        else:
            ops.gemm(dY, X, dW, M=Mo, N=No, K=M, a_kmajor=True, b_kmajor=True, Cin=dW, c_map=c_map)

    for li in range(nl - 1, -1, -1):
        attn, _, ff = tr.layers[li]
        w, sv = pw.layers[li], saved["layers"][li]
        F, Fp = w["F"], w["Fp"]
        dh2 = torch.empty(M, Fp, dtype=T, device=dev)
        ops.gemm(dres_c, w["W2p"], dh2, M=M, N=Fp, K=D, b_kmajor=True)
        gW2 = grad_of(ff.w_out.weight)
        wgrad(dres_c, sv.h2, gW2, D, F)
        if ws is None or ws.numel() < ops.ffmid_bwd_workspace_floats(F, Fp):
            ws = torch.empty(ops.ffmid_bwd_workspace_floats(F, Fp), device=dev)
        du = torch.empty(M, 2 * Fp, dtype=T, device=dev)
        dh1 = torch.empty(M, 2 * Fp, dtype=T, device=dev)
        gconv = grad_of(ff.conv_param()).view(-1) if ff.conv_param() is not None else None
        ops.ffmid_bwd(dh2, sv.h1, w["convw"], w["gamma_mid"], sv.m3, sv.r3, du, dh1,
                      grad_of(ff.norm_mid.gamma), gconv, ws, N, F, Fp, sv.p, sv.seed,
                      seed_dev=saved["salt"] if sv.p > 0 else None, drop_bits=sv.drop_bits, gh=sv.gh)
        del du, dh2
        dxn2 = torch.empty(M, D, dtype=T, device=dev)
        ops.gemm(dh1, w["W1p"], dxn2, M=M, N=D, K=2 * Fp, b_kmajor=True)
        gW1 = grad_of(ff.w_in.weight)
        wgrad(dh1, sv.xn2, gW1, 2 * Fp, D, c_map=w["dW1_cmap"])
        del dh1
        dx1 = torch.empty(M, D, device=dev)
        dx1_c = dx1 if T == torch.float32 else torch.empty(M, D, dtype=T, device=dev)
        ops.layernorm_bwd(dxn2, sv.x1, ff.norm_in.gamma.detach(), sv.m2, sv.r2, dres, dx1,
                          None if T == torch.float32 else dx1_c, grad_of(ff.norm_in.gamma), defer=cg)
        dyo = dx1_c
        if sv.po > 0:
            dyo = torch.empty(M, D, dtype=T, device=dev)
            ops.dropout_residual_bwd(dx1, dyo, sv.po, sv.so, seed_dev=saved["salt"])
        do = torch.empty(M, H * DIM_HEAD, dtype=T, device=dev)
        ops.gemm(dyo, w["Wo"], do, M=M, N=H * DIM_HEAD, K=D, b_kmajor=True)
        gWo = grad_of(attn.to_out[0].weight)
        wgrad(dyo, sv.o, gWo, D, H * DIM_HEAD)
        dq = torch.empty(M, H * DIM_HEAD, device=dev)
        dkv = torch.empty(2, M, DIM_HEAD, device=dev)
        dk, dv = dkv[0], dkv[1]
        delta = torch.empty(B, H, N, device=dev)
        ops.attn_bwd(sv.q, sv.k, sv.v, sv.abias, keymask, sv.o, do, sv.lse, delta, dq, dk, dv, dtable, B, N, H, ATTN_SCALE, P=prefix_rows(tr),
                     p=sv.pa, seed=sv.sa, seed_dev=saved["salt"] if sv.pa > 0 else None)
        dq_raw = torch.empty(M, H * DIM_HEAD, dtype=T, device=dev)
        dkv_raw = torch.empty(M, 2 * DIM_HEAD, dtype=T, device=dev)
        if T in _H16:
            ops.qk_norm_bwd2(dq, dk, dv, sv.q, sv.k, sv.q_raw, sv.kv_raw, attn.q_scale.detach(), attn.k_scale.detach(),
                             dq_raw, dkv_raw, grad_of(attn.q_scale), grad_of(attn.k_scale), H)
        else:
            ops.qk_norm_bwd(dq, dk, dv, sv.q_raw, sv.kv_raw, attn.q_scale.detach(), attn.k_scale.detach(),
                            dq_raw, dkv_raw, grad_of(attn.q_scale), grad_of(attn.k_scale), H)
        dxn = torch.empty(M, D, dtype=T, device=dev)
        kv16 = T in _H16
        tmp = torch.empty(M, D, dtype=T if kv16 else torch.float32, device=dev)
        ops.gemm(dq_raw, w["Wq"], dxn, M=M, N=D, K=H * DIM_HEAD, b_kmajor=True)
        ops.gemm(dkv_raw, w["Wkv"], tmp, M=M, N=D, K=2 * DIM_HEAD, b_kmajor=True, Cin=None if kv16 else dx1)
        gWq = grad_of(attn.to_q.weight)
        wgrad(dq_raw, sv.xn, gWq, H * DIM_HEAD, D)
        gWkv = grad_of(attn.to_kv.weight)
        wgrad(dkv_raw, sv.xc, gWkv, 2 * DIM_HEAD, D)
        dres = torch.empty(M, D, device=dev)
        dres_c = dres if T == torch.float32 else torch.empty(M, D, dtype=T, device=dev)
        last = li == 0
        ops.layernorm_bwd(dxn, sv.x, attn.norm.gamma.detach(), sv.m1, sv.r1, dx1 if kv16 else tmp, dres,
                          None if (T == torch.float32 or last) else dres_c, grad_of(attn.norm.gamma),
                          dx_scale=out_scale if last else 1.0, dres2=tmp if kv16 else None, defer=cg)
    cg.flush()
    if wg is not None:
        wg.flush()
    if dtable is not None and saved["rp"] is not None and not rp_cached:
        relpos_backward(tr, N, saved["rp"], dtable)
    return dres


def build_ids(model, all_token_ids: Sequence[torch.Tensor]) -> Tuple[torch.Tensor, List[int]]:
    parts, lens = [], []
    for seq, ids in zip(model.token_sequences, all_token_ids):
        ids = ids.reshape(ids.shape[0], -1)
        if seq.num_quantizers > 1:
            off = seq.codebook_size * (torch.arange(ids.shape[-1], device=ids.device) % seq.num_quantizers)
            ids = ids + off
        lens.append(ids.shape[-1])
        parts += [torch.full((ids.shape[0], 1), -2, device=ids.device, dtype=torch.int32), ids.to(torch.int32)]
    return torch.cat(parts, dim=1).contiguous(), lens


class PreparedIds:
    __slots__ = ("ids32", "lens")

    def __init__(self, ids32: torch.Tensor, lens: Sequence[int]):
        self.ids32, self.lens = ids32, list(lens)


def get_layout(model, B: int, lens: Sequence[int], device, final_rows_only: bool) -> SeqLayout:
    cache = model.__dict__.setdefault("_omlm_layouts", {})
    key = (B, tuple(lens), str(device), final_rows_only)
    if key not in cache:
        if len(cache) > 64:
            cache.clear()
        cache[key] = build_layout(B, lens, [s.num_quantizers for s in model.token_sequences], device, final_rows_only)
    return cache[key]


def embed_forward(model, ids32: torch.Tensor, lay: SeqLayout) -> torch.Tensor:
    B, N = ids32.shape
    D = model.dim
    x = torch.empty(B * N, D, device=ids32.device)
    pos = [e.weight.detach() for e in model.absolute_position_embeddings] if model.use_absolute_position_embeddings else None
    ops.embed_fwd(ids32, lay.seg, lay.posidx, [e.weight.detach() for e in model.embeddings],
                  [s.detach() for s in model.start_tokens], pos, x.view(B, N, D))
    return x


def embed_backward(model, ids32: torch.Tensor, lay: SeqLayout, dx: torch.Tensor, alpha: float):
    B, N = ids32.shape
    dpos = [grad_of(e.weight) for e in model.absolute_position_embeddings] if model.use_absolute_position_embeddings else None
    ops.embed_bwd(ids32, lay.seg, lay.posidx, [grad_of(e.weight) for e in model.embeddings],
                  [grad_of(s) for s in model.start_tokens], dpos, dx.view(B, N, -1), alpha)


def heads_forward(model, pw: PreparedWeights, y: torch.Tensor, y_lo: Optional[torch.Tensor], lay: SeqLayout, want: Sequence[bool]):
    D = model.dim
    out = []
    for s, seq in enumerate(model.token_sequences):
        if not want[s]:
            out.append(None)
            continue
        V1 = seq.codebook_size + 1
        ldV = ceil_to(V1, 8)
        n_s = lay.n_out[s]
        buf = torch.empty(lay.B if lay.final_only else lay.B * n_s, ldV, device=y.device)
        for qq in range(seq.num_quantizers):
            ent = lay.head_maps.get((s, qq))
            if ent is None:
                continue
            a_map, c_map, rows = ent
            if y_lo is not None:
                ops.gemm_planes16(y, y_lo, pw.heads[s][qq], pw.heads_lo[s][qq], buf, M=rows, N=V1, K=D, a_map=a_map, c_map=c_map, ldc=ldV,
                                  a_rows=y.shape[0], b_rows=V1)
                continue
            ops.gemm(y, pw.heads[s][qq], buf, M=rows, N=V1, K=D, a_map=a_map, c_map=c_map, ldc=ldV,
                     a_rows=y.shape[0], b_rows=V1)
        out.append(buf)
    return out


def heads_backward(model, pw: PreparedWeights, y: torch.Tensor, lay: SeqLayout, dlogits: Sequence[Optional[torch.Tensor]],
                   deferred: Optional[list] = None):
    D = model.dim
    dy = torch.zeros(y.shape[0], D, device=y.device)
    for s, seq in enumerate(model.token_sequences):
        dl = dlogits[s]
        if dl is None:
            continue
        V1 = seq.codebook_size + 1
        ldV = dl.shape[-1]
        gW = grad_of(model.logit_weights[s])
        for qq in range(seq.num_quantizers):
            ent = lay.head_maps.get((s, qq))
            if ent is None:
                continue
            a_map, c_map, rows = ent
            ops.gemm(dl, pw.heads[s][qq], dy, M=rows, N=D, K=ldV, b_kmajor=True, a_map=c_map, c_map=a_map,
                     a_rows=dl.shape[0], b_rows=V1)
            if deferred is not None and rows >= 1024:
                rp = ceil_to(rows, 64)
                gd = torch.empty(rp, dl.shape[-1], dtype=dl.dtype, device=dl.device)
                gy = torch.empty(rp, y.shape[-1], dtype=y.dtype, device=y.device)
                torch.index_select(dl, 0, c_map, out=gd[:rows])
                torch.index_select(y, 0, a_map, out=gy[:rows])
                if rp > rows:
                    gd[rows:].zero_(); gy[rows:].zero_()
                deferred.append((gd, gy, gW[qq], V1, D))
                continue
            ops.gemm(dl, y, gW[qq], M=V1, N=D, K=rows, a_kmajor=True, b_kmajor=True, a_map=c_map, b_map=a_map,
                     Cin=gW[qq], lda=ldV, a_rows=dl.shape[0], b_rows=y.shape[0])
    return dy


class ForwardState:
    __slots__ = ("model", "pw", "ids32", "lay", "trunk", "y", "B", "N", "logits", "labels", "lse_rows", "coefs")


def run_forward(model, all_token_ids, self_attn_mask, only_final: bool, save: bool, precision: str,
                want: Optional[Sequence[bool]] = None, final_rows_only: bool = False):
    tr = model.transformer
    require_gpu(model.start_tokens[0], "model parameters")
    ops.planes_begin()
    if isinstance(all_token_ids, PreparedIds):
        ids32, lens = all_token_ids.ids32, all_token_ids.lens
    else:
        ids32, lens = build_ids(model, all_token_ids)
    require_gpu(ids32, "token ids")
    B, N = ids32.shape
    lay = get_layout(model, B, lens, ids32.device, final_rows_only)
    pw = prepared_weights(model, precision) if not save else PreparedWeights(model, precision)
    keymask = None
    if self_attn_mask is not None:
        assert self_attn_mask.shape == (B, N), f"self_attn_mask must be [{B}, {N}]"
        keymask = self_attn_mask.to(torch.uint8).contiguous()
    x = embed_forward(model, ids32, lay)
    y, y_lo, tsaved = trunk_forward(tr, pw, x, keymask, B, N, save, model.training)
    nseq = len(model.token_sequences)
    if want is None:
        want = [(not only_final) or s == nseq - 1 for s in range(nseq)]
    logits = heads_forward(model, pw, y, y_lo, lay, want)
    st = None
    if save:
        st = ForwardState()
# ... 135 lines not shown
```

### open_musiclm_amd/hip.py

```python
from __future__ import annotations

import ctypes as C
import os
from typing import Optional

import torch

_HERE = os.path.dirname(os.path.abspath(__file__))
LIB_PATH = os.environ.get("OMLM_LIB_PATH") or os.path.join(_HERE, "libomlm_hip.so")

_lib: Optional[C.CDLL] = None

vp, i32, i64, f32, u64, f64 = C.c_void_p, C.c_int, C.c_longlong, C.c_float, C.c_ulonglong, C.c_double

SIGNATURES = {
    "omlm_version": [],
    "omlm_last_error": [],
    "omlm_set_error": [C.c_char_p],
    "omlm_gemm": [vp, vp, vp, vp, vp, vp, vp, i64, i64, i32, i32, i32, i32, i32, i32, i32, i32, i32, i32, i32, f32, vp, i64, vp],
    "omlm_gemm_tail_workspace_bytes": [i32, i32],
    "omlm_gemm_wgrad_group": [vp, i32, i32, i32, vp],
    "omlm_gemm_planes": [vp, i64, vp, i64, vp, vp, vp, vp, vp, i64, i64, i32, i32, i32, i32, i32, i32, i32, i32, i32, i32, f32, vp, i64, vp],
    "omlm_split_planes": [vp, vp, i64, i64, vp],
    "omlm_gemm_planes16": [vp, vp, vp, vp, vp, vp, vp, vp, vp, i64, i64, i32, i32, i32, i32, i32, i32, i32, i32, vp, i64, vp],
    "omlm_gemm_mx16": [vp, vp, i64, vp, vp, vp, i64, vp, vp, vp, i32, vp, i64, i64, i32, i32, i32, i32, i32, i32, i32, vp, i64, vp],
    "omlm_gemm_mx16_workspace_bytes": [i32, i32, i32],
    "omlm_layernorm_fwd_mx": [vp, vp, vp, vp, i64, vp, vp, vp, i32, i32, i32, f32, vp],
    "omlm_ffmid_fwd_mx": [vp, vp, vp, vp, vp, vp, vp, vp, i64, vp, vp, vp, i32, i32, i32, i32, f32, f32, u64, vp, vp, vp, vp],
    "omlm_quant_rows_mx": [vp, i32, vp],
    "omlm_layernorm_fwd_planes": [vp, vp, vp, vp, vp, vp, i32, i32, i32, f32, i32, vp],
    "omlm_ffmid_fwd_planes": [vp, vp, vp, vp, vp, vp, vp, vp, vp, vp, i32, i32, i32, i32, f32, f32, u64, vp, vp, vp, i32, vp],
    "omlm_layernorm_fwd": [vp, vp, vp, vp, vp, vp, i32, i32, i32, f32, i32, vp],
    "omlm_layernorm_bwd_workspace_bytes": [i32],
    "omlm_layernorm_bwd2": [vp, vp, vp, vp, vp, vp, vp, vp, vp, vp, vp, i32, i32, f32, i32, i32, vp],
    "omlm_qk_norm_fwd": [vp, vp, vp, vp, vp, vp, vp, i32, i32, i32, vp],
    "omlm_qk_norm_bwd": [vp, vp, vp, vp, vp, vp, vp, vp, vp, vp, vp, i32, i32, i32, vp],
    "omlm_gemm_qknorm": [vp, vp, vp, vp, i32, i32, vp, vp, i32, i32, i64, i64, i32, i32, i32, i32, i32, i32, i32, vp],
    "omlm_qk_norm_bwd2": [vp, vp, vp, vp, vp, vp, vp, vp, vp, vp, vp, vp, vp, i32, i32, i32, vp],
    "omlm_attn_bias_table_floats": [i32, i32, i32],
    "omlm_attn_bias_prepare": [vp, vp, i32, i32, i32, vp, vp, f32, f32, i32, vp],
    "omlm_attn_bias_prepare_group": [vp, vp, i32, i32, i32, i32, vp, vp, f32, f32, i32, i32, vp],
    "omlm_mqa_attn_fwd": [vp] * 8 + [i32, i32, i32, f32, i32, i32, i32, f32, u64, vp, vp],
    "omlm_mqa_attn_bwd": [vp] * 15 + [i32, i32, i32, f32, i32, i32, i32, f32, u64, vp, vp],
    "omlm_mqa_attn_bwd_workspace_bytes": [i32, i32, i32],
    "omlm_attn_dropout_keep": [vp, i32, i32, i32, f32, u64, vp, vp],
    "omlm_dropout_residual_fwd": [vp, vp, vp, i64, i32, f32, u64, vp, vp],
    "omlm_dropout_residual_bwd": [vp, vp, i64, i32, f32, u64, vp, i32, vp],
    "omlm_ffmid_fwd": [vp, vp, vp, vp, vp, vp, i32, i32, i32, i32, f32, f32, u64, vp, vp, vp, i32, vp],
    "omlm_ffmid_bwd_workspace_bytes": [i32, i32],
    "omlm_ffmid_bwd": [vp, vp, vp, vp, vp, vp, vp, vp, vp, vp, vp, i32, i32, i32, i32, f32, u64, vp, vp, vp, i32, vp],
    "omlm_colsum_accumulate": [vp, vp, i32, i32, i32, vp],
    "omlm_colsum_group": [vp, i32, vp],
    "omlm_ffmid_set_impl": [i32],
    "omlm_embed_gather_fwd": [vp, vp, vp, vp, vp, vp, i32, vp, i32, i32, i32, vp, vp, vp, vp],
    "omlm_embed_gather_bwd": [vp, vp, vp, vp, vp, vp, i32, vp, i32, i32, i32, f32, vp, vp, vp, vp],
    "omlm_prepare_train_batch": [vp, vp, vp, vp, vp, vp, i32, i32, i32, vp, i32, vp, vp, i32, vp],
    "omlm_cross_entropy_fwd": [vp, vp, vp, vp, i32, i32, i32, vp, vp],
    "omlm_cross_entropy_bwd": [vp, vp, vp, vp, f32, vp, i32, i32, i32, i32, i32, vp],
    "omlm_sumsq_accumulate": [vp, i64, vp, vp, vp],
    "omlm_adamw_clip_step": [vp, vp, vp, vp, vp, i64, f32, f32, f32, f32, f32, i32, f32, vp, f32, i32, i32, i32, vp, vp],
    "omlm_loss_scale_update": [vp, vp, f32, f32, i32, f32, f32, vp],
    "omlm_cast_pad": [vp, vp, i64, i32, i32, i32, i32, vp],
    "omlm_cast_pad_group": [vp, i32, i32, vp],
    "omlm_sample_topk_gumbel_at": [vp, vp, vp, vp, vp, i32, i32, i32, i32, f32, i32, vp],
    "omlm_sample_embed_at": [vp, vp, vp, vp, vp, i32, i32, i32, i32, f32, i32, vp, i64, i64, vp, i32, vp],
    "omlm_decode_step": [vp, vp, vp],
    "omlm_decode_advance": [vp, vp, vp],
    "omlm_relpos_first_fwd": [vp, vp, vp, vp, i32, i32, i32, vp],
    "omlm_relpos_first_bwd": [vp, vp, i32, i32, i32, vp],
    "omlm_bias_silu_fwd": [vp, vp, vp, vp, i64, i32, vp],
    "omlm_silu_bwd": [vp, vp, vp, i64, vp],
    "omlm_bias_add": [vp, vp, vp, i32, i32, i32, vp],
    "omlm_relpos_mlp_fwd": [vp] * 15 + [i32, i32, i32, i32, i32, vp],
    "omlm_relpos_mlp_bwd": [vp] * 19 + [i32, i32, i32, i32, i32, vp],
    "omlm_rvq_encode": [vp, vp, vp, vp, i32, i32, i32, i32, i32, vp],
    "omlm_nearest_centroid": [vp, vp, vp, i32, i32, i32, vp],
    "omlm_vq_accumulate": [vp, vp, i32, vp, vp, i32, i32, i32, vp],
    "omlm_vq_kmeans_update": [vp, vp, vp, vp, i32, i32, vp],
    "omlm_vq_ema_update": [vp, vp, vp, vp, vp, vp, vp, i32, i32, f32, f32, vp],
    "omlm_kmeans_pp_workspace_bytes": [i32, i32],
    "omlm_kmeans_pp_pick": [vp] * 9 + [i64, i32, i32, i32, i32, vp],
    "omlm_kmeans_pp_seed": [vp] * 9 + [i64, i32, i32, i32, i32, vp],
    "omlm_kmeans_minibatch_step": [vp] * 10 + [i32, i32, i32, i32, f64, f64, i32, vp],
    "omlm_kmeans_inertia": [vp, vp, vp, vp, i32, i32, i32, vp],
    "omlm_sample_topk_gumbel": [vp, vp, vp, i32, i32, i32, i32, f32, i32, vp],
    "omlm_probe_tr16": [vp, vp],
}
_RESTYPES = {"omlm_last_error": C.c_char_p, "omlm_gemm_tail_workspace_bytes": C.c_longlong, "omlm_gemm_mx16_workspace_bytes": C.c_longlong, "omlm_ffmid_bwd_workspace_bytes": C.c_longlong,
             "omlm_attn_bias_table_floats": C.c_longlong, "omlm_mqa_attn_bwd_workspace_bytes": C.c_longlong,
             "omlm_layernorm_bwd_workspace_bytes": C.c_longlong, "omlm_kmeans_pp_workspace_bytes": C.c_longlong,
             "omlm_set_error": None}


class HipLibraryMissing(RuntimeError):
    pass


def lib() -> C.CDLL:
    global _lib
    if _lib is None:
        if not os.path.exists(LIB_PATH):
            raise HipLibraryMissing(
                f"{LIB_PATH} not found: build it with `python -c 'import __graft_entry__ as g; g.build()'` "
                "(or `make -C open_musiclm_amd/csrc`). There is no CPU fallback for the MI355X hot path.")
        l = C.CDLL(LIB_PATH)
        for name, args in SIGNATURES.items():
            fn = getattr(l, name)
            fn.argtypes = args
            fn.restype = _RESTYPES.get(name, C.c_int)
        _lib = l
    return _lib


def stream_ptr() -> int:
    return torch.cuda.current_stream().cuda_stream


def ptr(t: Optional[torch.Tensor]):
    if t is None:
        return None
    return t.data_ptr()


def call(name: str, *args):
    rc = getattr(lib(), name)(*args)
    if rc != 0:
        msg = lib().omlm_last_error()
        raise RuntimeError(f"{name} failed (rc={rc}): {msg.decode() if msg else '?'}")


def require_gpu(t: torch.Tensor, what: str = "tensor"):
    if not t.is_cuda:
        raise RuntimeError(
            f"open_musiclm_amd: {what} is on {t.device}; the TokenConditionedTransformer path only runs on an "
            "MI355X through libomlm_hip.so (no CPU fallback). Move the model and inputs to 'cuda'.")
    cur = torch.cuda.current_device()
    if t.device.index != cur:
        raise RuntimeError(f"open_musiclm_amd: {what} lives on cuda:{t.device.index} but the current device is cuda:{cur}; "
                           "call torch.cuda.set_device(LOCAL_RANK) and keep the model and its inputs on that device")
```

### open_musiclm_amd/ops.py

```python
from __future__ import annotations

import ctypes as C
import os
import weakref
from typing import Optional, Sequence

import torch

from . import hip
from .hip import call, ptr, stream_ptr

F32, BF16, F16 = 0, 1, 2
_CODES = {torch.float32: F32, torch.bfloat16: BF16, torch.float16: F16}
H16 = (torch.bfloat16, torch.float16)


def dcode(dtype: torch.dtype) -> int:
    try:
        return _CODES[dtype]
    except KeyError:
        raise TypeError(f"unsupported operand dtype {dtype}") from None


def tdtype(code: int) -> torch.dtype:
    return {F32: torch.float32, BF16: torch.bfloat16, F16: torch.float16}[code]


def _chk(t: torch.Tensor, name: str):
    hip.require_gpu(t, name)
    if not t.is_contiguous():
        raise ValueError(f"{name} must be contiguous")


_X3_PLANES = os.environ.get("OMLM_X3_PLANES", "1") == "1"
_X3_MIN_MACS = 1 << 26
_PLANES = {}
_PLANE_SCOPE = [0]


def planes_begin():
    _PLANES.clear()
    _PLANE_SCOPE[0] = 1


def planes_end():
    _PLANES.clear()
    _PLANE_SCOPE[0] = 0


def operand_planes(t: torch.Tensor, rows: int, ld: int):
    n = int(rows) * int(ld)
    key = id(t)
    scoped = _PLANE_SCOPE[0] > 0
    if scoped:
        ent = _PLANES.get(key)
        if ent is not None and ent[0]() is t and ent[1] == t._version and ent[2] == (t.data_ptr(), n):
            return ent[3], ent[4]
    pe = (n + 7) // 8 * 8
    buf = torch.empty(2 * pe, dtype=torch.bfloat16, device=t.device)
    call("omlm_split_planes", ptr(t), ptr(buf), n, pe, stream_ptr())
    if scoped:
        try:
            ref = weakref.ref(t, lambda _r, k=key: _PLANES.pop(k, None))
            _PLANES[key] = (ref, t._version, (t.data_ptr(), n), buf, pe * 2)
        except TypeError:
            pass
    return buf, pe * 2


_TAIL_WS = {}
_TAIL_WS_BYTES = int(os.environ.get("OMLM_GEMM_TAIL_WS_MB", "64")) << 20


def tail_workspace(device: torch.device):
    if _TAIL_WS_BYTES <= 0:
        return None, 0
    idx = device.index if device.index is not None else torch.cuda.current_device()
    key = (idx, torch.cuda.current_stream(device).cuda_stream)
    buf = _TAIL_WS.get(key)
    if buf is None:
        buf = _TAIL_WS[key] = torch.empty(_TAIL_WS_BYTES // 4, device=device)
    return ptr(buf), _TAIL_WS_BYTES


def gemm(A: torch.Tensor, B: torch.Tensor, C_: torch.Tensor, *, M: int, N: int, K: int,
         lda: Optional[int] = None, ldb: Optional[int] = None, ldc: Optional[int] = None,
         a_kmajor: bool = False, b_kmajor: bool = False, Cin: Optional[torch.Tensor] = None,
         ldcin: Optional[int] = None, a_map=None, b_map=None, c_map=None, alpha: float = 1.0,
         a_rows: Optional[int] = None, b_rows: Optional[int] = None, planes: bool = True):
    hip.require_gpu(A, "A")
    assert A.dtype == B.dtype, (A.dtype, B.dtype)
    lda = lda if lda is not None else A.shape[-1]
    ldb = ldb if ldb is not None else B.shape[-1]
    ldc = ldc if ldc is not None else C_.shape[-1]
    if Cin is not None:
        assert Cin.dtype == torch.float32
        ldcin = ldcin if ldcin is not None else Cin.shape[-1]
    a_rows = a_rows if a_rows is not None else A.numel() // lda
    b_rows = b_rows if b_rows is not None else B.numel() // ldb
    ws, wsb = tail_workspace(A.device) if (A.dtype in H16 or A.dtype == torch.float32) else (None, 0)
    if (A.dtype == torch.float32 and planes and _X3_PLANES and M * N * K >= _X3_MIN_MACS and not (a_kmajor and a_map is not None)
            and not (b_kmajor and b_map is not None) and (a_kmajor and b_kmajor or K % 8 == 0)):
        pa, sa = operand_planes(A, a_rows, lda)
        pb, sb = operand_planes(B, b_rows, ldb)
        call("omlm_gemm_planes", ptr(pa), sa, ptr(pb), sb, ptr(C_), ptr(Cin), ptr(a_map), ptr(b_map), ptr(c_map),
             a_rows, b_rows, M, N, K, lda, ldb, ldc, ldcin or 0, int(a_kmajor), int(b_kmajor), dcode(C_.dtype), float(alpha),
             ws, wsb, stream_ptr())
        return
    call("omlm_gemm", ptr(A), ptr(B), ptr(C_), ptr(Cin), ptr(a_map), ptr(b_map), ptr(c_map),
         a_rows, b_rows, M, N, K, lda, ldb, ldc, ldcin or 0, int(a_kmajor), int(b_kmajor),
         dcode(A.dtype), dcode(C_.dtype), float(alpha), ws, wsb, stream_ptr())


def gemm_planes16(A, A_lo, B, B_lo, C_, C_lo=None, *, M: int, N: int, K: int, Cin: Optional[torch.Tensor] = None, a_map=None, c_map=None,
                  ldc: Optional[int] = None, a_rows: Optional[int] = None, b_rows: Optional[int] = None):
    hip.require_gpu(A, "A")
    assert A.dtype in H16 and A_lo.dtype == A.dtype and B.dtype == A.dtype and B_lo.dtype == A.dtype
    assert A_lo.shape == A.shape and B_lo.shape == B.shape
    if C_lo is None:
        assert C_.dtype == torch.float32 and (Cin is None or Cin.dtype == torch.float32)
    else:
        assert C_.dtype == A.dtype and C_lo.dtype == A.dtype and C_lo.shape == C_.shape and Cin is None
    lda, ldb = A.shape[-1], B.shape[-1]
    ldc = ldc if ldc is not None else C_.shape[-1]
    ws, wsb = tail_workspace(A.device)
    call("omlm_gemm_planes16", ptr(A), ptr(A_lo), ptr(B), ptr(B_lo), ptr(C_), ptr(C_lo), ptr(Cin), ptr(a_map), ptr(c_map),
         a_rows if a_rows is not None else A.numel() // lda, b_rows if b_rows is not None else B.numel() // ldb,
         M, N, K, lda, ldb, ldc, Cin.shape[-1] if Cin is not None else 0, dcode(A.dtype), ws, wsb, stream_ptr())


class Fp8Planes:
    __slots__ = ("planes", "scale", "rows", "ld")

    def __init__(self, rows: int, ld: int, device, zero: bool = True):
        self.rows, self.ld = int(rows), int(ld)
        rp = (self.rows + 255) // 256 * 256
        self.planes = (torch.zeros if zero else torch.empty)(2, rp, 2 * self.ld, dtype=torch.uint8, device=device)
        self.scale = (torch.full((rp,), 127, dtype=torch.uint8, device=device) if zero else torch.empty(rp, dtype=torch.uint8, device=device))

    @property
    def stride(self) -> int:
        return self.planes.shape[1] * self.planes.shape[2]


def gemm_mx16(A, A8: Fp8Planes, B, B8: Fp8Planes, C_, C_lo=None, *, M: int, N: int, K: int, Cin: Optional[torch.Tensor] = None):
    hip.require_gpu(A, "A")
    assert A.dtype == torch.float16 and B.dtype == torch.float16
    lda, ldb = A.shape[-1], B.shape[-1]
    assert A8.ld == lda and B8.ld == ldb and A8.rows >= M and B8.rows >= N
    if C_lo is None:
        assert C_.dtype == torch.float32 and (Cin is None or Cin.dtype == torch.float32)
    else:
        assert C_.dtype == A.dtype and C_lo.dtype in (A.dtype, torch.uint8) and C_lo.shape == C_.shape and Cin is None
    ws, wsb = tail_workspace(A.device)
    call("omlm_gemm_mx16", ptr(A), ptr(A8.planes), A8.stride, ptr(A8.scale), ptr(B), ptr(B8.planes), B8.stride, ptr(B8.scale),
         ptr(C_), ptr(C_lo), int(C_lo is not None and C_lo.dtype == torch.uint8), ptr(Cin), A.numel() // lda, B.numel() // ldb, M, N, K, lda, ldb, C_.shape[-1],
         Cin.shape[-1] if Cin is not None else 0, ws, wsb, stream_ptr())


class _DescGroup:
    desc = entry = dtype = None

    def __init__(self):
        self.items = []

    def _fields(self, item):
        return [ptr(v) if v is None or isinstance(v, torch.Tensor) else v for v in item]

    def flush(self, *args):
        if not self.items:
            return
        arr = (self.desc * len(self.items))(*[self.desc(*self._fields(it)) for it in self.items])
        call(self.entry, C.cast(arr, C.c_void_p), len(arr), *args, *([] if self.dtype is None else [dcode(self.dtype)]), stream_ptr())
        self.items = []


class _WgradDesc(C.Structure):
    _fields_ = [("A", C.c_void_p), ("B", C.c_void_p), ("C", C.c_void_p), ("c_map", C.c_void_p),
                ("M", C.c_int), ("N", C.c_int), ("K", C.c_int), ("lda", C.c_int), ("ldb", C.c_int), ("ldc", C.c_int)]


class WgradGroup(_DescGroup):
    desc, entry = _WgradDesc, "omlm_gemm_wgrad_group"

    def add(self, dY: torch.Tensor, X: torch.Tensor, dW: torch.Tensor, *, M: int, N: int, K: int, c_map=None):
        hip.require_gpu(dY, "dY")
        assert dY.dtype in H16 and X.dtype == dY.dtype and dW.dtype == torch.float32
        assert self.dtype in (None, dY.dtype), "one operand type per group"
        self.dtype = dY.dtype
        self.items.append((dY, X, dW, c_map, M, N, K, dY.shape[-1], X.shape[-1], dW.shape[-1]))

    def flush(self, splits: int = 0):
        super().flush(int(splits))


class _CastDesc(C.Structure):
    _fields_ = [("src", C.c_void_p), ("dst", C.c_void_p), ("R", C.c_int), ("C", C.c_int), ("ld_src", C.c_int), ("ld_dst", C.c_int),
                ("transpose", C.c_int), ("lo", C.c_int)]


class CastPadGroup(_DescGroup):
    desc, entry = _CastDesc, "omlm_cast_pad_group"

    def add(self, src, dst, R, C_, ld_src, ld_dst, transpose=False, lo=False):
        hip.require_gpu(src, "src")
        assert src.dtype == torch.float32 and self.dtype in (None, dst.dtype), "fp32 sources, one output type per group"
        self.dtype = dst.dtype
        self.items.append((src, dst, int(R), int(C_), int(ld_src), int(ld_dst), int(bool(transpose)), int(bool(lo))))


def layernorm_fwd(x, gamma, y, xcast, mean, rstd, eps=1e-5):
    M, D = x.shape
    call("omlm_layernorm_fwd", ptr(x), ptr(gamma), ptr(y), ptr(xcast), ptr(mean), ptr(rstd),
         M, D, y.shape[-1], float(eps), dcode(y.dtype), stream_ptr())


def layernorm_fwd_planes(x, gamma, y, y_lo, mean, rstd, eps=1e-5):
    M, D = x.shape
    assert y.dtype in H16 and y_lo.dtype == y.dtype and y_lo.shape == y.shape
    call("omlm_layernorm_fwd_planes", ptr(x), ptr(gamma), ptr(y), ptr(y_lo), ptr(mean), ptr(rstd),
         M, D, y.shape[-1], float(eps), dcode(y.dtype), stream_ptr())


def layernorm_fwd_mx(x, gamma, y, P: "Fp8Planes", mean, rstd, eps=1e-5):
    M, D = x.shape
    assert y.dtype == torch.float16 and P.ld == y.shape[-1] and P.rows >= M
    call("omlm_layernorm_fwd_mx", ptr(x), ptr(gamma), ptr(y), ptr(P.planes), P.stride, ptr(P.scale), ptr(mean), ptr(rstd),
         M, D, y.shape[-1], float(eps), stream_ptr())


class _QuantDesc(C.Structure):
    _fields_ = [("src", C.c_void_p), ("dst8", C.c_void_p), ("lo_stride", C.c_longlong), ("scale8", C.c_void_p),
                ("R", C.c_int), ("C", C.c_int), ("ld_src", C.c_int), ("ld8", C.c_int)]


class QuantRowsGroup(_DescGroup):
    desc, entry = _QuantDesc, "omlm_quant_rows_mx"

    def add(self, src, P: "Fp8Planes", row0: int, R: int, C_: int, ld_src: int):
        hip.require_gpu(src, "src")
        assert src.dtype == torch.float32 and row0 + R <= P.rows and C_ <= 2 * P.ld
        self.items.append((src, P, int(row0), int(R), int(C_), int(ld_src)))

    def _fields(self, item):
        src, P, row0, R, C_, ld_src = item
        pitch = 2 * P.ld
        return ptr(src), P.planes.data_ptr() + row0 * pitch, P.stride, P.scale.data_ptr() + row0, R, C_, ld_src, pitch


_LN_WS = {}


def _ln_workspace(D: int, device) -> torch.Tensor:
    key = (D, str(device))
    if key not in _LN_WS:
        _LN_WS[key] = torch.empty(int(hip.lib().omlm_layernorm_bwd_workspace_bytes(D)) // 4, device=device)
    return _LN_WS[key]


class _ColsumDesc(C.Structure):
    _fields_ = [("part", C.c_void_p), ("out", C.c_void_p), ("P", C.c_int), ("C", C.c_int), ("ldp", C.c_int)]


class ColsumGroup(_DescGroup):
    desc, entry = _ColsumDesc, "omlm_colsum_group"

    def add(self, part: torch.Tensor, out: torch.Tensor, P: int, C_: int, ldp: int):
        self.items.append((part, out, int(P), int(C_), int(ldp)))


def layernorm_bwd(dy, x, gamma, mean, rstd, dres, dx, dxcast, dgamma, dx_scale=1.0, dres2=None, defer: Optional["ColsumGroup"] = None):
    M, D = x.shape
    code = dcode(dxcast.dtype) if dxcast is not None else (dcode(dres2.dtype) if dres2 is not None else F32)
    assert dres2 is None or dcode(dres2.dtype) == code, "dres2 must have the cast type"
    deferred = dgamma is not None and defer is not None
    rows = min(M, 2048)
    if deferred:
        ws = torch.empty(rows * D, device=x.device)
    else:
        ws = _ln_workspace(D, x.device) if dgamma is not None else None
    call("omlm_layernorm_bwd2", ptr(dy), ptr(x), ptr(gamma), ptr(mean), ptr(rstd), ptr(dres), ptr(dres2), ptr(dx),
         ptr(dxcast), ptr(None if deferred else dgamma), ptr(ws), M, D, float(dx_scale), code, dcode(dy.dtype), stream_ptr())
    if deferred:
        defer.add(ws, dgamma, rows, D, D)


def qk_norm_fwd(q_raw, kv_raw, q_scale, k_scale, q, k, v, H):
    call("omlm_qk_norm_fwd", ptr(q_raw), ptr(kv_raw), ptr(q_scale), ptr(k_scale), ptr(q), ptr(k), ptr(v),
         q_raw.shape[0], H, dcode(q.dtype), stream_ptr())


def qk_norm_bwd(dq, dk, dv, q_raw, kv_raw, q_scale, k_scale, dq_raw, dkv_raw, dq_scale, dk_scale, H):
    call("omlm_qk_norm_bwd", ptr(dq), ptr(dk), ptr(dv), ptr(q_raw), ptr(kv_raw), ptr(q_scale), ptr(k_scale),
         ptr(dq_raw), ptr(dkv_raw), ptr(dq_scale), ptr(dk_scale), q_raw.shape[0], H, dcode(dq_raw.dtype), stream_ptr())


_DBIAS_WS = {}
_DBIAS_RETIRED = []


def gemm_qknorm(A, B, C_, scale, norm_out, groups, *, M, N, K, C2=None, c2_col0=0):
    hip.require_gpu(A, "A")
    assert A.dtype in H16 and B.dtype == A.dtype and C_.dtype == A.dtype and norm_out.dtype == torch.float32 and scale.dtype == torch.float32
    assert C2 is None or C2.dtype == A.dtype
    call("omlm_gemm_qknorm", ptr(A), ptr(B), ptr(C_), ptr(C2), int(c2_col0), C2.shape[-1] if C2 is not None else 0, ptr(scale), ptr(norm_out),
         norm_out.shape[-1] if norm_out.dim() > 1 else 1, int(groups), A.numel() // A.shape[-1], B.numel() // B.shape[-1], M, N, K,
         A.shape[-1], B.shape[-1], C_.shape[-1], dcode(A.dtype), stream_ptr())


def qk_norm_bwd2(dq, dk, dv, q, k, qn, kn, q_scale, k_scale, dq_raw, dkv_raw, dq_scale, dk_scale, H):
    call("omlm_qk_norm_bwd2", ptr(dq), ptr(dk), ptr(dv), ptr(q), ptr(k), ptr(qn), ptr(kn), ptr(q_scale), ptr(k_scale),
         ptr(dq_raw), ptr(dkv_raw), ptr(dq_scale), ptr(dk_scale), q.shape[0], H, dcode(dq_raw.dtype), stream_ptr())


class AttnBias:

    def __init__(self, table: Optional[torch.Tensor], N: int, H: int, device=None, q_scale=None, k_scale=None,
                 qk_bound: float = 0.0, scale: float = 8.0, half: bool = False, _tableT: Optional[torch.Tensor] = None, _P: int = 0):
        self.table, self.N, self.H, self.P = table, N, H, _P
        dev = table.device if table is not None else device
        if _tableT is not None:
            self.tableT = _tableT
            return
        self.tableT = torch.empty(int(hip.lib().omlm_attn_bias_table_floats(N, H, 0)), device=dev)
        call("omlm_attn_bias_prepare", ptr(table), ptr(self.tableT), N, H, table.shape[-1] if table is not None else 0,
             ptr(q_scale), ptr(k_scale), float(qk_bound), float(scale), 15 if half else 0, stream_ptr())

    @staticmethod
    def group(table: Optional[torch.Tensor], N: int, H: int, device, q_scales, k_scales, scale: float = 8.0, half: bool = False, P: int = 0):
        L = len(q_scales)
        dev = table.device if table is not None else device
        buf = torch.empty(L, int(hip.lib().omlm_attn_bias_table_floats(N, H, P)), device=dev)
        outs = (C.c_void_p * L)(*[buf[l].data_ptr() for l in range(L)])
        qs = (C.c_void_p * L)(*[t.data_ptr() for t in q_scales])
        ks = (C.c_void_p * L)(*[t.data_ptr() for t in k_scales])
        for t in list(q_scales) + list(k_scales):
            hip.require_gpu(t, "scale")
        call("omlm_attn_bias_prepare_group", ptr(table), C.cast(outs, C.c_void_p), L, N, H, table.shape[-1] if table is not None else 0,
             C.cast(qs, C.c_void_p), C.cast(ks, C.c_void_p), 0.0, float(scale), 15 if half else 0, int(P), stream_ptr())
        return [AttnBias(table, N, H, dev, _tableT=buf[l], _P=P) for l in range(L)]


def _attn_tables(bias, N, H, P, device):
    if isinstance(bias, AttnBias):
        if bias.P != P:
            raise ValueError(f"attention with P = {P} handed an AttnBias prepared for P = {bias.P}")
        return bias.table, bias.tableT
    return bias, (AttnBias(bias, N, H, device).tableT if P == 0 else None)


def _dbias_workspace(B: int, N: int, H: int, device) -> torch.Tensor:
    n = int(hip.lib().omlm_mqa_attn_bwd_workspace_bytes(B, N, H)) // 4
    key = str(device)
    ws = _DBIAS_WS.get(key)
    if ws is None or ws.numel() < n:
        if ws is not None:
            _DBIAS_RETIRED.append(ws)
        ws = _DBIAS_WS[key] = torch.empty(n, device=device, dtype=torch.float32)
    return ws


def attn_fwd(q, k, v, bias, keymask, out, lse, B, N, H, scale, P=0, p=0.0, seed=0, seed_dev=None):
    table, tableT = _attn_tables(bias, N, H, P, q.device)
    call("omlm_mqa_attn_fwd", ptr(q), ptr(k), ptr(v), ptr(table), ptr(tableT), ptr(keymask), ptr(out), ptr(lse), B, N, H, float(scale),
         table.shape[-1] if table is not None else 0, dcode(q.dtype), int(P), float(p), int(seed), ptr(seed_dev), stream_ptr())


def attn_bwd(q, k, v, bias, keymask, out, dout, lse, delta, dq, dk, dv, dbias, B, N, H, scale, P=0, workspace=True, p=0.0, seed=0,
             seed_dev=None):
    table, tableT = _attn_tables(bias, N, H, P, q.device)
    ws = _dbias_workspace(B, N, H, q.device) if dbias is not None and workspace else None
    ld = table.shape[-1] if table is not None else (dbias.shape[-1] if dbias is not None else 0)
    call("omlm_mqa_attn_bwd", ptr(q), ptr(k), ptr(v), ptr(table), ptr(tableT), ptr(keymask), ptr(out), ptr(dout), ptr(lse), ptr(delta), ptr(dq),
         ptr(dk), ptr(dv), ptr(dbias), ptr(ws), B, N, H, float(scale), ld, dcode(q.dtype), int(P), float(p), int(seed), ptr(seed_dev),
         stream_ptr())


def attn_dropout_keep(B, N, H, p, seed, seed_dev=None, device=None) -> torch.Tensor:
    keep = torch.empty(B, H, N, N, dtype=torch.uint8, device=device if device is not None else seed_dev.device)
    call("omlm_attn_dropout_keep", ptr(keep), B, N, H, float(p), int(seed), ptr(seed_dev), stream_ptr())
    return keep


def dropout_residual_fwd(x, y, x1, p, seed, seed_dev=None):
    call("omlm_dropout_residual_fwd", ptr(x), ptr(y), ptr(x1), x.shape[0], x.shape[1], float(p), int(seed), ptr(seed_dev), stream_ptr())


def dropout_residual_bwd(dx1, dy, p, seed, seed_dev=None):
    call("omlm_dropout_residual_bwd", ptr(dx1), ptr(dy), dx1.shape[0], dx1.shape[1], float(p), int(seed), ptr(seed_dev), dcode(dy.dtype),
         stream_ptr())


def pack_conv_taps(convw: torch.Tensor, F: int, Fp: int) -> torch.Tensor:
    out = torch.zeros(3, 2 * Fp, device=convw.device, dtype=torch.float32)
    out[:, :F] = convw[:F].t()
    out[:, Fp:Fp + F] = convw[F:].t()
    return out


def pad_vector(v: torch.Tensor, n: int) -> torch.Tensor:
    out = torch.zeros(n, device=v.device, dtype=torch.float32)
    out[: v.numel()] = v
    return out


def ffmid_fwd(h1, convw, gamma, h2, mean, rstd, nseq, F, Fp, p, seed, eps=1e-5, seed_dev=None, drop_bits=None, gh=None):
    assert convw.shape == (3, 2 * Fp) and gamma.numel() == Fp
    assert convw.dtype == h1.dtype and gamma.dtype == h1.dtype, "taps / gamma travel in the operand dtype of h1"
    call("omlm_ffmid_fwd", ptr(h1), ptr(convw), ptr(gamma), ptr(h2), ptr(mean), ptr(rstd),
         h1.shape[0], nseq, F, Fp, float(eps), float(p), int(seed), ptr(seed_dev), ptr(drop_bits), ptr(gh), dcode(h1.dtype),
         stream_ptr())


def ffmid_fwd_planes(h1, h1_lo, convw, convw_lo, gamma, gamma_lo, h2, h2_lo, mean, rstd, nseq, F, Fp, p, seed, eps=1e-5, seed_dev=None,
                     drop_bits=None, gh=None):
    assert convw.shape == (3, 2 * Fp) and gamma.numel() == Fp and h1.dtype in H16
    for t in (h1_lo, convw, convw_lo, gamma, gamma_lo, h2, h2_lo):
        assert t.dtype == h1.dtype, "every plane travels in the operand dtype of h1"
    assert h1_lo.shape == h1.shape and h2_lo.shape == h2.shape and convw_lo.shape == convw.shape
    call("omlm_ffmid_fwd_planes", ptr(h1), ptr(h1_lo), ptr(convw), ptr(convw_lo), ptr(gamma), ptr(gamma_lo), ptr(h2), ptr(h2_lo), ptr(mean),
         ptr(rstd), h1.shape[0], nseq, F, Fp, float(eps), float(p), int(seed), ptr(seed_dev), ptr(drop_bits), ptr(gh), dcode(h1.dtype),
         stream_ptr())


def ffmid_fwd_mx(h1, h1_lo, convw, convw_lo, gamma, gamma_lo, h2, P: "Fp8Planes", mean, rstd, nseq, F, Fp, p, seed, eps=1e-5, seed_dev=None,
                 drop_bits=None, gh=None):
    assert convw.shape == (3, 2 * Fp) and gamma.numel() == Fp and h1.dtype == torch.float16 and h1_lo.dtype == torch.uint8
    for t in (convw, convw_lo, gamma, gamma_lo, h2):
        assert t.dtype == h1.dtype, "every plane travels in the operand dtype of h1"
    assert h1_lo.shape == h1.shape and convw_lo.shape == convw.shape and P.ld == Fp and P.rows >= h1.shape[0]
    call("omlm_ffmid_fwd_mx", ptr(h1), ptr(h1_lo), ptr(convw), ptr(convw_lo), ptr(gamma), ptr(gamma_lo), ptr(h2), ptr(P.planes), P.stride,
         ptr(P.scale), ptr(mean), ptr(rstd), h1.shape[0], nseq, F, Fp, float(eps), float(p), int(seed), ptr(seed_dev), ptr(drop_bits), ptr(gh),
         stream_ptr())


def ffmid_set_impl(impl: int):
    call("omlm_ffmid_set_impl", int(impl))


def ffmid_bwd_workspace_floats(F, Fp) -> int:
    return int(hip.lib().omlm_ffmid_bwd_workspace_bytes(F, Fp)) // 4


def ffmid_bwd(dh2, h1, convw, gamma, mean, rstd, du_tmp, dh1, dgamma, dconv, workspace, nseq, F, Fp, p, seed, seed_dev=None,
              drop_bits=None, gh=None):
    assert convw.shape == (3, 2 * Fp) and gamma.numel() == Fp
    assert convw.dtype == h1.dtype and gamma.dtype == h1.dtype, "taps / gamma travel in the operand dtype of h1"
    call("omlm_ffmid_bwd", ptr(dh2), ptr(h1), ptr(convw), ptr(gamma), ptr(mean), ptr(rstd), ptr(du_tmp), ptr(dh1),
         ptr(dgamma), ptr(dconv), ptr(workspace), h1.shape[0], nseq, F, Fp, float(p), int(seed), ptr(seed_dev), ptr(drop_bits),
         ptr(gh), dcode(h1.dtype), stream_ptr())


def _ptr_array(tensors: Sequence[Optional[torch.Tensor]]):
    arr = (C.c_void_p * len(tensors))()
    for i, t in enumerate(tensors):
        arr[i] = ptr(t) if t is not None else None
    return arr


_INDEX_ERR = {}


def index_error_flag(device) -> torch.Tensor:
    key = str(device)
    if key not in _INDEX_ERR:
        _INDEX_ERR[key] = torch.zeros(1, dtype=torch.int32, device=device)
    return _INDEX_ERR[key]


def raise_on_index_error(device):
    flag = _INDEX_ERR.get(str(device))
    if flag is None:
        return
    v = int(flag.item())
    if v:
        flag.zero_()
        what = [n for b, n in ((1, "token id >= embedding rows"), (2, "position >= absolute position rows"), (4, "label >= vocabulary")) if v & b]
        raise IndexError("open_musiclm_amd: " + ", ".join(what) + " (rows were skipped; check codebook sizes / the token store)")


def _rows_array(tensors):
    if tensors is None:
        return None
    return (C.c_longlong * len(tensors))(*[int(t.shape[0]) if t is not None else 0 for t in tensors])


def embed_fwd(ids, seg, posidx, tables, starts, pos_tables, out):
    B, N = ids.shape
    D = out.shape[-1]
    pos_arr = _ptr_array(pos_tables) if pos_tables is not None else None
    call("omlm_embed_gather_fwd", ptr(ids), ptr(seg), ptr(posidx), _ptr_array(tables), _ptr_array(starts),
         pos_arr, len(tables), ptr(out), B, N, D, _rows_array(tables), _rows_array(pos_tables), ptr(index_error_flag(out.device)),
         stream_ptr())


def embed_bwd(ids, seg, posidx, dtables, dstarts, dpos_tables, dx, alpha):
    B, N = ids.shape
    D = dx.shape[-1]
    pos_arr = _ptr_array(dpos_tables) if dpos_tables is not None else None
    call("omlm_embed_gather_bwd", ptr(ids), ptr(seg), ptr(posidx), _ptr_array(dtables), _ptr_array(dstarts),
         pos_arr, len(dtables), ptr(dx), B, N, D, float(alpha), _rows_array(dtables), _rows_array(dpos_tables),
         ptr(index_error_flag(dx.device)), stream_ptr())


def prepare_train_batch(raw_ids, eos_ids, quantizers, codebooks, pad_id, scores, n_drop, want_labels):
    n = len(raw_ids)
    B, dev = raw_ids[0].shape[0], raw_ids[0].device
    for t in raw_ids:
        hip.require_gpu(t, "token ids")
        assert t.dtype == torch.int64 and t.dim() == 2 and t.is_contiguous() and t.shape[0] == B
    lens = [int(t.shape[1]) for t in raw_ids]
    N = sum(l + 1 for l in lens) + (n - 1)
    ids32 = torch.empty(B, N, dtype=torch.int32, device=dev)
    keymask = torch.empty(B, N, dtype=torch.uint8, device=dev)
    labels = [torch.empty(B, l + 1, dtype=torch.int32, device=dev) if w else None for l, w in zip(lens, want_labels)]
    arr_i = lambda v: (C.c_int * n)(*[int(x) for x in v])
    call("omlm_prepare_train_batch", _ptr_array(raw_ids), _ptr_array(labels), arr_i(lens), arr_i(eos_ids), arr_i(quantizers), arr_i(codebooks),
         n, B, int(pad_id), ptr(scores), int(n_drop), ptr(ids32), ptr(keymask), N, stream_ptr())
    return ids32, keymask, labels, [l + 1 for l in lens[:-1]] + [lens[-1]]


def ce_fwd(logits, labels, row_lse, nll_sum, V):
    R, ld = logits.shape
    call("omlm_cross_entropy_fwd", ptr(logits), ptr(labels), ptr(row_lse), ptr(nll_sum), R, V, ld,
         ptr(index_error_flag(logits.device)), stream_ptr())


def ce_bwd(logits, labels, row_lse, gscale, coef, dlogits, V):
    R, ld = logits.shape
    call("omlm_cross_entropy_bwd", ptr(logits), ptr(labels), ptr(row_lse), ptr(gscale), float(coef), ptr(dlogits),
         R, V, ld, dlogits.shape[-1], dcode(dlogits.dtype), stream_ptr())


def sumsq_accumulate(g, out, partials=None):
    call("omlm_sumsq_accumulate", ptr(g), g.numel(), ptr(out), ptr(partials), stream_ptr())


def adamw_clip_step(p, g, m, v, p16, *, lr, beta1, beta2, eps, wd, step, gscale, gnorm_sq, max_norm,
                    decoupled, zero_grad, ls_state=None):
    call("omlm_adamw_clip_step", ptr(p), ptr(g), ptr(m), ptr(v), ptr(p16), p.numel(), float(lr), float(beta1),
         float(beta2), float(eps), float(wd), int(step), float(gscale), ptr(gnorm_sq), float(max_norm or 0.0),
         int(decoupled), int(zero_grad), dcode(p16.dtype) if p16 is not None else BF16, ptr(ls_state), stream_ptr())


def loss_scale_update(ls_state, gnorm_sq, *, growth=2.0, backoff=0.5, interval=2000, scale_min=1.0, scale_max=65536.0):
    call("omlm_loss_scale_update", ptr(ls_state), ptr(gnorm_sq), float(growth), float(backoff), int(interval), float(scale_min),
         float(scale_max), stream_ptr())


def cast_pad(src, dst, R, C_, ld_src, ld_dst):
    call("omlm_cast_pad", ptr(src), ptr(dst), R, C_, ld_src, ld_dst, dcode(dst.dtype), stream_ptr())


def colsum_accumulate(part, out, P, C_, ldp):
    call("omlm_colsum_accumulate", ptr(part), ptr(out), P, C_, ldp, stream_ptr())


def relpos_first_fwd(w0, b0, pre, z, n, Hd, x0=0):
    call("omlm_relpos_first_fwd", ptr(w0), ptr(b0), ptr(pre), ptr(z), n, Hd, int(x0), stream_ptr())


def relpos_first_bwd(ds, dw0, n, Hd, x0=0):
    call("omlm_relpos_first_bwd", ptr(ds), ptr(dw0), n, Hd, int(x0), stream_ptr())


def bias_silu_fwd(a, b, pre, z, R, C_):
    call("omlm_bias_silu_fwd", ptr(a), ptr(b), ptr(pre), ptr(z), R, C_, stream_ptr())


def silu_bwd(dz, pre, ds, total):
    call("omlm_silu_bwd", ptr(dz), ptr(pre), ptr(ds), total, stream_ptr())


def bias_add(a, b, out, R, C_, ld):
    call("omlm_bias_add", ptr(a), ptr(b), ptr(out), R, C_, ld, stream_ptr())


def relpos_mlp_fwd(w0, b0, W1, b1, W2, b2, W3, b3, saves, table, n, Hd, H, ldb, x0=0):
    sv = saves if saves is not None else [None] * 6
    call("omlm_relpos_mlp_fwd", ptr(w0), ptr(b0), ptr(W1), ptr(b1), ptr(W2), ptr(b2), ptr(W3), ptr(b3), *[ptr(t) for t in sv], ptr(table),
         int(n), int(Hd), int(H), int(ldb), int(x0), stream_ptr())


def relpos_mlp_bwd(dtable, W1, W2, W3, saves, scratch, grads, n, Hd, H, ldb, x0=0):
    call("omlm_relpos_mlp_bwd", ptr(dtable), ptr(W1), ptr(W2), ptr(W3), *[ptr(t) for t in saves], ptr(scratch), *[ptr(g) for g in grads],
         int(n), int(Hd), int(H), int(ldb), int(x0), stream_ptr())


def rvq_encode(x, codebooks_T, indices, residual_out, n, D, C_, nstage, idx_stride=None):
    call("omlm_rvq_encode", ptr(x), ptr(codebooks_T), ptr(indices), ptr(residual_out), n, D, C_, nstage, int(idx_stride or 0), stream_ptr())


def nearest_centroid(x, centroids_T, indices, n, D, C_):
    hip.require_gpu(x, "x")
# ... 78 lines not shown
```

Before: 1153 samples/s.

## Group independent small GEMMs into one persistent launch and shrink ffmid bwd scratch

Adds a grouped persistent GEMM kernel that walks the tiles of up to four independent problems in one launch. Attention backward uses it to run the dq and dkv input-gradient GEMMs together, and the forward q/kv projections with the l2-norm epilogue can do the same. The aim is to cut launch count and fill the GPU better when each GEMM alone has too few tiles. It also adds a query that sizes the ffmid backward scratch buffer to the path actually taken, which avoids allocating the full M*2*Fp buffer when the fused path only needs M*2 floats. The cost is extra kernel code and some fallback complexity.

```diff
diff --git a/include/omlm.h b/include/omlm.h
--- a/include/omlm.h
+++ b/include/omlm.h
@@ -66,6 +66,7 @@
                           void* h2, void* h2_lo, float* mean, float* rstd, int M, int nseq, int F, int Fp, float eps, float p,
                           unsigned long long seed, const unsigned long long* seed_dev, unsigned char* drop_bits, void* gh, int dtype, void* stream);
 long long omlm_ffmid_bwd_workspace_bytes(int F, int Fp);
+long long omlm_ffmid_bwd_scratch_bytes(int M, int Fp, int have_gh, float p, int have_drop_bits, int dtype);
 int omlm_ffmid_bwd(const void* dh2, const void* h1, const void* convw, const void* gamma, const float* mean,
                    const float* rstd, void* du_tmp, void* dh1, float* dgamma, float* dconv, float* workspace,
                    int M, int nseq, int F, int Fp, float p, unsigned long long seed,
@@ -131,6 +132,12 @@
     int M, N, K, lda, ldb, ldc;
 } omlm_gemm_wgrad_desc;
 int omlm_gemm_wgrad_group(const omlm_gemm_wgrad_desc* problems, int count, int splits, int dtype, void* stream);
+typedef struct omlm_gemm_group_desc {
+    const void* A; const void* B; void* C; void* C2; const float* scale; float* norm_out;
+    long long a_rows, b_rows;
+    int M, N, K, lda, ldb, ldc, ldc2, c2_col0, ldnorm, groups;
+} omlm_gemm_group_desc;
+int omlm_gemm_group(const omlm_gemm_group_desc* problems, int count, int epi, int b_kmajor, int dtype, void* workspace, long long workspace_bytes, void* stream);
 
 int omlm_relpos_first_fwd(const float* w0, const float* b0, float* pre, float* z, int n, int Hd, int x0, void* stream);
 int omlm_relpos_first_bwd(const float* ds, float* dw0, int n, int Hd, int x0, void* stream);
diff --git a/open_musiclm_amd/csrc/ffmid.hip b/open_musiclm_amd/csrc/ffmid.hip
--- a/open_musiclm_amd/csrc/ffmid.hip
+++ b/open_musiclm_amd/csrc/ffmid.hip
@@ -550,6 +550,11 @@
 extern "C" long long omlm_ffmid_bwd_workspace_bytes(int F, int Fp) {
     return (long long)sizeof(float) * ((long long)FF_BWD1_BLOCKS * Fp + (long long)FF_BWD2_STRIPS * 2 * F * 3);
 }
+extern "C" long long omlm_ffmid_bwd_scratch_bytes(int M, int Fp, int have_gh, float p, int have_drop_bits, int dtype) {
+    if (M <= 0 || Fp <= 0) return 0;
+    if (ffmid_impl() == 1 && ffmid2_supported(Fp) && have_gh && (p == 0.f || have_drop_bits)) return (long long)M * 2 * sizeof(float);
+    return (long long)M * 2 * Fp * (dtype == OMLM_DT_F32 ? 4 : 2);
+}
 #endif
 
 #if !OMLM_FP16
diff --git a/open_musiclm_amd/csrc/gemm.hip b/open_musiclm_amd/csrc/gemm.hip
--- a/open_musiclm_amd/csrc/gemm.hip
+++ b/open_musiclm_amd/csrc/gemm.hip
@@ -487,7 +487,200 @@
 }
 
 
+#define OMLM_PGROUP_MAX 4
+struct PersistGroupArgs { int n; int start[OMLM_PGROUP_MAX + 1]; GemmArgs p[OMLM_PGROUP_MAX]; };
+
+template <int BM_, int BN_, int WM_, int WN_, bool B_KMAJ, typename TOUT, int EPI, bool CIN = false>
+__device__ __forceinline__ void gemm_persist_walk(const GemmArgs& g, int lin, const int G, char* smem) {
+    constexpr bool A_KMAJ = false;
+    constexpr int NWN = BN_ / WN_, NWAVES = (BM_ / WM_) * NWN;
+    constexpr int MI = WM_ / 32, NJ = WN_ / 32;
+    constexpr int A_BYTES = BM_ * BK * 2, B_BYTES = BN_ * BK * 2, STAGE = A_BYTES + B_BYTES;
+    constexpr int UA = (BM_ / 8) / NWAVES, UB = (BN_ / 8) / NWAVES;
+    constexpr int PATCH = 32 * (WN_ + 4) * 4;
+    static_assert((NWAVES - 1) * PATCH <= STAGE, "all but the last wave's patch must fit inside one stage");
+    constexpr int GROUP = OMLM_SUPER_ROWS / BM_;
+    constexpr int VEC = sizeof(TOUT) == 2 ? 8 : 4, NSTORE = MI * (32 / (64 / (WN_ / VEC)));
+
+    const int tiles_m = (g.M + BM_ - 1) / BM_, tiles_n = (g.N + BN_ - 1) / BN_;
+    const int total = tiles_m * tiles_n;
+    const int nk = g.K / BK;
+    const int lane = threadIdx.x & 63;
+    const int wave = __builtin_amdgcn_readfirstlane(threadIdx.x >> 6);
+    const int wm = (wave / NWN) * WM_, wn = (wave % NWN) * WN_;
+    const dma_rsrc rsA = make_dma_rsrc(g.A, (unsigned long long)g.a_rows * g.lda * 2);
+    const dma_rsrc rsB = make_dma_rsrc(g.B, (unsigned long long)g.b_rows * g.ldb * 2);
+    const unsigned smem_lds = (unsigned)(size_t)LDS_PTR(char, smem);
+
+    auto origin = [&](int l, int& m0, int& n0) {
+        const int bid = xcd_logical_id(l, total);
+        const int gsz = GROUP * tiles_n;
+        const int grp = bid / gsz, first_m = grp * GROUP;
+        const int rows_in = min(GROUP, tiles_m - first_m);
+        m0 = (first_m + (bid - grp * gsz) % rows_in) * BM_;
+        n0 = ((bid - grp * gsz) / rows_in) * BN_;
+    };
+    auto piece = [&](int l, const unsigned (&va)[UA], const unsigned (&vb)[UB], int k0, unsigned stage_lds, bool live) {
+        if (l < UA) {
+            const int b = wave + NWAVES * l;
+            dma_issue_s(rsA, stage_lds + (unsigned)(b * 1024), live ? va[l] : OOB_OFF,
+                        A_KMAJ ? (unsigned)k0 * (unsigned)(g.lda * 2) : (unsigned)(k0 * 2));
+        } else {
+            const int b = wave + NWAVES * (l - UA);
+            dma_issue_s(rsB, stage_lds + (unsigned)A_BYTES + (unsigned)(b * 1024), live ? vb[l - UA] : OOB_OFF,
+                        B_KMAJ ? (unsigned)k0 * (unsigned)(g.ldb * 2) : (unsigned)(k0 * 2));
+        }
+    };
+
+    if (lin >= total) return;
+    int m0, n0;
+    origin(lin, m0, n0);
+    unsigned va[UA], vb[UB];
+    {
+        DmaStagerT<A_KMAJ, BM_, NWAVES> sa;
+        DmaStagerT<B_KMAJ, BN_, NWAVES> sb;
+        sa.init(nullptr, g.lda, g.M, m0, wave, lane);
+        sb.init(nullptr, g.ldb, g.N, n0, wave, lane);
+#pragma unroll
+        for (int i = 0; i < UA; ++i) va[i] = sa.vfast[i];
+#pragma unroll
+        for (int i = 0; i < UB; ++i) vb[i] = sb.vfast[i];
+    }
+    int par = 0;
+#pragma unroll
+    for (int l = 0; l < UA + UB; ++l) piece(l, va, vb, 0, smem_lds, true);
+    bool counted = false;
+
+    for (;;) {
+        const int lin_n = lin + G;
+        const bool has_next = lin_n < total;
+        int m0n = m0, n0n = n0;
+        if (has_next) origin(lin_n, m0n, n0n);
+        unsigned van[UA], vbn[UB];
+        {
+            DmaStagerT<A_KMAJ, BM_, NWAVES> sa;
+            DmaStagerT<B_KMAJ, BN_, NWAVES> sb;
+            sa.init(nullptr, g.lda, g.M, m0n, wave, lane);
+            sb.init(nullptr, g.ldb, g.N, n0n, wave, lane);
+#pragma unroll
+            for (int i = 0; i < UA; ++i) van[i] = sa.vfast[i];
+#pragma unroll
+            for (int i = 0; i < UB; ++i) vbn[i] = sb.vfast[i];
+        }
+        f32x16 acc[MI][NJ];
+#pragma unroll
+        for (int i = 0; i < MI; ++i)
+#pragma unroll
+            for (int j = 0; j < NJ; ++j)
+#pragma unroll
+                for (int e = 0; e < 16; ++e) acc[i][j][e] = 0.f;
+        {
+            h16x8 a[2][MI], b[2][NJ];
+            bool pending = false;
+            constexpr int MPS = MI * NJ, NLOAD = UA + UB;
+            constexpr int SPREAD = 2;
+            constexpr int STRIDE = (SPREAD * MPS) / NLOAD > 0 ? (SPREAD * MPS) / NLOAD : 1;
+            for (int kt = 0; kt < nk; ++kt) {
+                const int cur = (par + kt) & 1;
+                if (kt == 0 && counted) asm volatile("s_waitcnt vmcnt(%0)" :: "n"(NSTORE) : "memory");
+                else asm volatile("s_waitcnt vmcnt(0)" ::: "memory");
+                __syncthreads();
+                const bool last = kt + 1 == nk;
+                const bool live = !last || has_next;
+                const unsigned nxt = smem_lds + (unsigned)((cur ^ 1) * STAGE);
+                const int knext = last ? 0 : (kt + 1) * BK;
+                const char* As = smem + cur * STAGE;
+                const char* Bs = As + A_BYTES;
+                auto phase = [&](const int ph, const int fi, const bool mul) {
+#pragma unroll
+                    for (int i = 0; i < MI; ++i)
+#pragma unroll
+                        for (int j = 0; j < NJ; ++j) {
+                            if (mul) acc[i][j] = OMLM_MFMA_32x32x16(a[fi][i], b[fi][j], acc[i][j]);
+                            const int midx = ph * MPS + i * NJ + j;
+                            if (midx % STRIDE == 0 && midx / STRIDE < NLOAD) {
+                                const int l = midx / STRIDE;
+                                __builtin_amdgcn_sched_barrier(0);
+                                unsigned v;
+                                if (l < UA) v = last ? van[l] : va[l]; else v = last ? vbn[l - UA] : vb[l - UA];
+                                {
+                                    unsigned one_a[UA], one_b[UB];
+#pragma unroll
+                                    for (int x = 0; x < UA; ++x) one_a[x] = v;
+#pragma unroll
+                                    for (int x = 0; x < UB; ++x) one_b[x] = v;
+                                    piece(l, one_a, one_b, knext, nxt, live);
+                                }
+                                __builtin_amdgcn_sched_barrier(0);
+                            }
+                        }
+                };
+#pragma unroll
+                for (int i = 0; i < MI; ++i) a[0][i] = read_frag<A_KMAJ>(As, wm + 32 * i, 0, lane);
+#pragma unroll
+                for (int j = 0; j < NJ; ++j) b[0][j] = read_frag<B_KMAJ>(Bs, wn + 32 * j, 0, lane);
+                __builtin_amdgcn_sched_barrier(0);
+                phase(0, 1, pending);
+                __builtin_amdgcn_sched_barrier(0);
+#pragma unroll
+                for (int st = 0; st < 3; ++st) {
+#pragma unroll
+                    for (int i = 0; i < MI; ++i) a[(st + 1) & 1][i] = read_frag<A_KMAJ>(As, wm + 32 * i, st + 1, lane);
+#pragma unroll
+                    for (int j = 0; j < NJ; ++j) b[(st + 1) & 1][j] = read_frag<B_KMAJ>(Bs, wn + 32 * j, st + 1, lane);
+                    __builtin_amdgcn_sched_barrier(0);
+                    phase(st + 1, st & 1, true);
+                    __builtin_amdgcn_sched_barrier(0);
+                }
+                pending = true;
+            }
+            if (pending) {
+#pragma unroll
+                for (int i = 0; i < MI; ++i)
+#pragma unroll
+                    for (int j = 0; j < NJ; ++j) acc[i][j] = OMLM_MFMA_32x32x16(a[1][i], b[1][j], acc[i][j]);
+            }
+        }
+        const int cur_last = (par + nk - 1) & 1;
+        if (!has_next) asm volatile("s_waitcnt vmcnt(0)" ::: "memory");
+        __syncthreads();
+        float* patch = wave < NWAVES - 1 ? (float*)(smem + cur_last * STAGE + wave * PATCH) : (float*)(smem + 2 * STAGE);
+        GemmArgs ge = g;
+        ge.c_map = nullptr;
+        if constexpr (!CIN) ge.Cin = nullptr;
+        tile_epilogue<MI, NJ, WN_, TOUT, EPI, false>(ge, acc, smem, m0, n0, wm, wn, wave, lane, false, patch);
+        if (!has_next) break;
+        counted = m0 + BM_ <= g.M && n0 + BN_ <= g.N;
+        par = (par + nk) & 1;
+        lin = lin_n; m0 = m0n; n0 = n0n;
+#pragma unroll
+        for (int i = 0; i < UA; ++i) va[i] = van[i];
+#pragma unroll
+        for (int i = 0; i < UB; ++i) vb[i] = vbn[i];
+    }
+}
+
+template <bool B_KMAJ, typename TOUT, int EPI>
+__global__ __launch_bounds__(256) void gemm_persist_group_kernel(PersistGroupArgs ga) {
+    extern __shared__ __attribute__((aligned(16))) char smem[];
+    const int G = gridDim.x;
+    bool walked = false;
+    for (int p = 0; p < ga.n; ++p) {
+        const int s0 = ga.start[p], s1 = ga.start[p + 1];
+        const int behind = s0 - (int)blockIdx.x;
+        const int first = (int)blockIdx.x + (behind > 0 ? (behind + G - 1) / G * G : 0);
+        if (first >= s1) continue;
+        if (walked) __syncthreads();
+        gemm_persist_walk<128, 128, 64, 64, B_KMAJ, TOUT, EPI>(ga.p[p], first - s0, G, smem);
+        walked = true;
+    }
+}
+
+
 #ifdef OMLM_ISA_ONLY
+template __global__ void gemm_persist_group_kernel<false, h16_t, 1>(PersistGroupArgs);
+template __global__ void gemm_persist_group_kernel<true, h16_t, 0>(PersistGroupArgs);
+template __global__ void gemm_bf16_tile_persist_kernel<128, 128, 64, 64, false, true, h16_t, false>(GemmArgs);
 template __global__ void gemm_bf16_tile_persist_kernel<256, 256, 128, 64, false, false, h16_t, false>(GemmArgs);
 template __global__ void gemm_bf16_tile_persist_kernel<256, 256, 128, 64, false, true, h16_t, false>(GemmArgs);
 template __global__ void gemm_bf16_tile_persist_kernel<256, 256, 128, 64, false, false, float, true>(GemmArgs);
@@ -886,6 +1079,93 @@
     return omlm_post_launch("omlm_gemm_qknorm");
 }
 
+struct omlm_gemm_group_desc {
+    const void* A; const void* B; void* C; void* C2; const float* scale; float* norm_out;
+    long long a_rows, b_rows;
+    int M, N, K, lda, ldb, ldc, ldc2, c2_col0, ldnorm, groups;
+};
+#if OMLM_FP16
+#define OMLM_SIBLING(name) name##_h
+#else
+#define OMLM_SIBLING(name) name
+extern "C" int omlm_gemm_group_h(const omlm_gemm_group_desc* d, int count, int epi, int b_kmajor, int dtype, void* workspace, long long workspace_bytes, void* stream);
+#endif
+extern "C" int OMLM_API(omlm_gemm_group)(const omlm_gemm_group_desc* d, int count, int epi, int b_kmajor, int dtype, void* workspace,
+                                         long long workspace_bytes, void* stream) {
+    if (count <= 0) return OMLM_OK;
+    OMLM_CHECK_ARG(d, "gemm_group: null descriptor array");
+#if !OMLM_FP16
+    if (dtype == OMLM_DT_F16) return omlm_gemm_group_h(d, count, epi, b_kmajor, 1, workspace, workspace_bytes, stream);
+#endif
+    OMLM_CHECK_ARG(dtype == 1, "gemm_group: operand dtype 1 (bf16) or 2 (fp16)");
+    OMLM_CHECK_ARG(epi == 0 || epi == 1, "gemm_group: epi 0 (plain) or 1 (l2-norm)");
+    OMLM_CHECK_ARG(!(epi == 1 && b_kmajor), "gemm_group: the l2-norm form takes row-major B");
+    const int slots = 2 * gemm_persist_slots();
+    bool grouped = count >= 2 && count <= OMLM_PGROUP_MAX && slots > 0;
+    long long total = 0;
+    for (int i = 0; i < count; ++i) {
+        const omlm_gemm_group_desc& q = d[i];
+        if (q.M <= 0 || q.N <= 0 || q.K <= 0 || q.K % BK != 0) grouped = false;
+        if (epi == 0 && !(q.K <= 512 && q.N <= 1024)) grouped = false;
+        if (q.M > 0 && q.N > 0) total += (long long)((q.M + 127) / 128) * ((q.N + 127) / 128);
+    }
+    if (total <= slots || total > 0x3FFFFFFF) grouped = false;
+    if (!grouped) {
+        for (int i = 0; i < count; ++i) {
+            const omlm_gemm_group_desc& q = d[i];
+            const int rc = epi == 1
+                ? OMLM_SIBLING(omlm_gemm_qknorm)(q.A, q.B, q.C, q.C2, q.c2_col0, q.ldc2, q.scale, q.norm_out, q.ldnorm, q.groups, q.a_rows, q.b_rows,
+                                             q.M, q.N, q.K, q.lda, q.ldb, q.ldc, 1, stream)
+                : OMLM_SIBLING(omlm_gemm)(q.A, q.B, q.C, nullptr, nullptr, nullptr, nullptr, q.a_rows, q.b_rows, q.M, q.N, q.K, q.lda, q.ldb, q.ldc, 0,
+                                      0, b_kmajor, 1, 1, 1.0f, workspace, workspace_bytes, stream);
+            if (rc != OMLM_OK) return rc;
+        }
+        return OMLM_OK;
+    }
+    PersistGroupArgs ga;
+    memset(&ga, 0, sizeof(ga));
+    ga.n = count;
+    int start = 0;
+    for (int i = 0; i < count; ++i) {
+        const omlm_gemm_group_desc& q = d[i];
+        OMLM_CHECK_ARG(q.A && q.B && q.C, "gemm_group: null operand");
+        OMLM_CHECK_ARG((q.lda % 8) == 0 && (q.ldb % 8) == 0 && ((uintptr_t)q.A % 16) == 0 && ((uintptr_t)q.B % 16) == 0,
+                       "gemm_group: 16-byte aligned operands, pitches multiples of 8");
+        OMLM_CHECK_ARG((unsigned long long)q.a_rows * q.lda * 2 < 0xFFFFFFF0ull && (unsigned long long)q.b_rows * q.ldb * 2 < 0xFFFFFFF0ull,
+                       "gemm_group: operand exceeds the 4 GiB window");
+        if (b_kmajor) OMLM_CHECK_ARG(q.ldb >= ((q.N + 7) / 8) * 8, "gemm_group: k-major B: row pitch shorter than N padded to 8");
+        if (epi == 1) {
+            OMLM_CHECK_ARG(q.scale && q.norm_out, "gemm_group: null scale / norm_out");
+            OMLM_CHECK_ARG((q.N % 64) == 0 && q.groups >= 0 && q.groups * 64 <= q.N && q.ldnorm >= q.groups, "gemm_group: N must be whole 64-wide heads");
+            OMLM_CHECK_ARG((q.ldc % 8) == 0 && ((uintptr_t)q.C % 16) == 0, "gemm_group: 16-byte aligned C, pitch a multiple of 8");
+            OMLM_CHECK_ARG(!q.C2 || ((q.c2_col0 % 64) == 0 && (q.ldc2 % 8) == 0 && ((uintptr_t)q.C2 % 16) == 0), "gemm_group: second output");
+        }
+        GemmArgs& g = ga.p[i];
+        g.A = q.A; g.B = q.B; g.C = q.C; g.a_rows = q.a_rows; g.b_rows = q.b_rows; g.M = q.M; g.N = q.N; g.K = q.K;
+        g.lda = q.lda; g.ldb = q.ldb; g.ldc = q.ldc; g.alpha = 1.f; g.kt_per_split = q.K / BK;
+        if (epi == 1) {
+            g.epi_scale = q.scale; g.epi_norm = q.norm_out; g.epi_groups = q.groups; g.epi_ldnorm = q.ldnorm;
+            g.C2 = q.C2; g.c2_col0 = q.c2_col0; g.ldc2 = q.ldc2;
+        }
+        ga.start[i] = start;
+        start += ((q.M + 127) / 128) * ((q.N + 127) / 128);
+    }
+    for (int i = count; i <= OMLM_PGROUP_MAX; ++i) ga.start[i] = start;
+    constexpr size_t LDSP = 2 * (size_t)(128 + 128) * BK * 2 + 32 * (64 + 4) * 4;
+    auto kq = gemm_persist_group_kernel<false, h16_t, 1>;
+    auto kn = gemm_persist_group_kernel<false, h16_t, 0>;
+    auto kk = gemm_persist_group_kernel<true, h16_t, 0>;
+    static bool attr = false;
+    if (!attr) {
+        (void)hipFuncSetAttribute((const void*)kq, hipFuncAttributeMaxDynamicSharedMemorySize, (int)LDSP);
+        (void)hipFuncSetAttribute((const void*)kn, hipFuncAttributeMaxDynamicSharedMemorySize, (int)LDSP);
+        (void)hipFuncSetAttribute((const void*)kk, hipFuncAttributeMaxDynamicSharedMemorySize, (int)LDSP);
+        attr = true;
+    }
+    hipLaunchKernelGGL(epi == 1 ? kq : (b_kmajor ? kk : kn), dim3(slots), dim3(256), LDSP, as_stream(stream), ga);
+    return omlm_post_launch("omlm_gemm_group");
+}
+
 #if !OMLM_FP16
 extern "C" int omlm_gemm_planes16_h(const void* A, const void* A_lo, const void* B, const void* B_lo, void* C, void* C_lo, const float* Cin,
                                     const int* a_map, const int* c_map, long long a_rows, long long b_rows, int M, int N, int K,
diff --git a/open_musiclm_amd/engine.py b/open_musiclm_amd/engine.py
--- a/open_musiclm_amd/engine.py
+++ b/open_musiclm_amd/engine.py
@@ -472,8 +472,9 @@
             qn = torch.empty(M, H, device=dev)
             kn = torch.empty(M, device=dev)
             q_raw, kv_raw = qn, kn
-            ops.gemm_qknorm(xn, w["Wq"], q, attn.q_scale.detach(), qn, H, M=M, N=H * DIM_HEAD, K=D)
-            ops.gemm_qknorm(xc, w["Wkv"], k, attn.k_scale.detach(), kn, 1, M=M, N=2 * DIM_HEAD, K=D, C2=v, c2_col0=DIM_HEAD)
+            ops.gemm_qknorm(xn, w["Wq"], q, attn.q_scale.detach(), qn, H, M=M, N=H * DIM_HEAD, K=D,
+                            rider=dict(A=xc, B=w["Wkv"], C=k, scale=attn.k_scale.detach(), norm_out=kn, groups=1, M=M, N=2 * DIM_HEAD, K=D,
+                                       C2=v, c2_col0=DIM_HEAD))
         else:
             q_raw = torch.empty(M, H * DIM_HEAD, device=dev)
             kv_raw = torch.empty(M, 2 * DIM_HEAD, device=dev)
@@ -606,7 +607,7 @@
         wgrad(dres_c, sv.h2, gW2, D, F)
         if ws is None or ws.numel() < ops.ffmid_bwd_workspace_floats(F, Fp):
             ws = torch.empty(ops.ffmid_bwd_workspace_floats(F, Fp), device=dev)
-        du = torch.empty(M, 2 * Fp, dtype=T, device=dev)
+        du = torch.empty(ops.ffmid_bwd_scratch_elems(M, Fp, T, sv.p, sv.drop_bits is not None, sv.gh is not None), dtype=T, device=dev)
         dh1 = torch.empty(M, 2 * Fp, dtype=T, device=dev)
         gconv = grad_of(ff.conv_param()).view(-1) if ff.conv_param() is not None else None
         ops.ffmid_bwd(dh2, sv.h1, w["convw"], w["gamma_mid"], sv.m3, sv.r3, du, dh1,
@@ -647,8 +648,12 @@
         dxn = torch.empty(M, D, dtype=T, device=dev)
         kv16 = T in _H16
         tmp = torch.empty(M, D, dtype=T if kv16 else torch.float32, device=dev)
-        ops.gemm(dq_raw, w["Wq"], dxn, M=M, N=D, K=H * DIM_HEAD, b_kmajor=True)
-        ops.gemm(dkv_raw, w["Wkv"], tmp, M=M, N=D, K=2 * DIM_HEAD, b_kmajor=True, Cin=None if kv16 else dx1)
+        if kv16:
+            ops.gemm(dq_raw, w["Wq"], dxn, M=M, N=D, K=H * DIM_HEAD, b_kmajor=True,
+                     rider=dict(A=dkv_raw, B=w["Wkv"], C=tmp, M=M, N=D, K=2 * DIM_HEAD))
+        else:
+            ops.gemm(dq_raw, w["Wq"], dxn, M=M, N=D, K=H * DIM_HEAD, b_kmajor=True)
+            ops.gemm(dkv_raw, w["Wkv"], tmp, M=M, N=D, K=2 * DIM_HEAD, b_kmajor=True, Cin=dx1)
         gWq = grad_of(attn.to_q.weight)
         wgrad(dq_raw, sv.xn, gWq, H * DIM_HEAD, D)
         gWkv = grad_of(attn.to_kv.weight)
diff --git a/open_musiclm_amd/hip.py b/open_musiclm_amd/hip.py
--- a/open_musiclm_amd/hip.py
+++ b/open_musiclm_amd/hip.py
@@ -20,6 +20,7 @@
     "omlm_gemm": [vp, vp, vp, vp, vp, vp, vp, i64, i64, i32, i32, i32, i32, i32, i32, i32, i32, i32, i32, i32, f32, vp, i64, vp],
     "omlm_gemm_tail_workspace_bytes": [i32, i32],
     "omlm_gemm_wgrad_group": [vp, i32, i32, i32, vp],
+    "omlm_gemm_group": [vp, i32, i32, i32, i32, vp, i64, vp],
     "omlm_gemm_planes": [vp, i64, vp, i64, vp, vp, vp, vp, vp, i64, i64, i32, i32, i32, i32, i32, i32, i32, i32, i32, i32, f32, vp, i64, vp],
     "omlm_split_planes": [vp, vp, i64, i64, vp],
     "omlm_gemm_planes16": [vp, vp, vp, vp, vp, vp, vp, vp, vp, i64, i64, i32, i32, i32, i32, i32, i32, i32, i32, vp, i64, vp],
@@ -48,6 +49,7 @@
     "omlm_dropout_residual_bwd": [vp, vp, i64, i32, f32, u64, vp, i32, vp],
     "omlm_ffmid_fwd": [vp, vp, vp, vp, vp, vp, i32, i32, i32, i32, f32, f32, u64, vp, vp, vp, i32, vp],
     "omlm_ffmid_bwd_workspace_bytes": [i32, i32],
+    "omlm_ffmid_bwd_scratch_bytes": [i32, i32, i32, f32, i32, i32],
     "omlm_ffmid_bwd": [vp, vp, vp, vp, vp, vp, vp, vp, vp, vp, vp, i32, i32, i32, i32, f32, u64, vp, vp, vp, i32, vp],
     "omlm_colsum_accumulate": [vp, vp, i32, i32, i32, vp],
     "omlm_colsum_group": [vp, i32, vp],
@@ -86,7 +88,7 @@
     "omlm_sample_topk_gumbel": [vp, vp, vp, i32, i32, i32, i32, f32, i32, vp],
     "omlm_probe_tr16": [vp, vp],
 }
-_RESTYPES = {"omlm_last_error": C.c_char_p, "omlm_gemm_tail_workspace_bytes": C.c_longlong, "omlm_gemm_mx16_workspace_bytes": C.c_longlong, "omlm_ffmid_bwd_workspace_bytes": C.c_longlong,
+_RESTYPES = {"omlm_last_error": C.c_char_p, "omlm_gemm_tail_workspace_bytes": C.c_longlong, "omlm_gemm_mx16_workspace_bytes": C.c_longlong, "omlm_ffmid_bwd_workspace_bytes": C.c_longlong, "omlm_ffmid_bwd_scratch_bytes": C.c_longlong,
              "omlm_attn_bias_table_floats": C.c_longlong, "omlm_mqa_attn_bwd_workspace_bytes": C.c_longlong,
              "omlm_layernorm_bwd_workspace_bytes": C.c_longlong, "omlm_kmeans_pp_workspace_bytes": C.c_longlong,
              "omlm_set_error": None}
diff --git a/open_musiclm_amd/ops.py b/open_musiclm_amd/ops.py
--- a/open_musiclm_amd/ops.py
+++ b/open_musiclm_amd/ops.py
@@ -83,13 +83,43 @@
     return ptr(buf), _TAIL_WS_BYTES
 
 
+class _GemmGroupDesc(C.Structure):
+    _fields_ = [("A", C.c_void_p), ("B", C.c_void_p), ("C", C.c_void_p), ("C2", C.c_void_p), ("scale", C.c_void_p), ("norm_out", C.c_void_p),
+                ("a_rows", C.c_longlong), ("b_rows", C.c_longlong),
+                ("M", C.c_int), ("N", C.c_int), ("K", C.c_int), ("lda", C.c_int), ("ldb", C.c_int), ("ldc", C.c_int), ("ldc2", C.c_int),
+                ("c2_col0", C.c_int), ("ldnorm", C.c_int), ("groups", C.c_int)]
+
+
+def _gemm_group(descs, epi: int, b_kmajor: bool, dtype, device):
+    ws, wsb = tail_workspace(device)
+    arr = (_GemmGroupDesc * len(descs))(*descs)
+    call("omlm_gemm_group", C.cast(arr, C.c_void_p), len(descs), int(epi), int(b_kmajor), dcode(dtype), ws, wsb, stream_ptr())
+
+
 def gemm(A: torch.Tensor, B: torch.Tensor, C_: torch.Tensor, *, M: int, N: int, K: int,
          lda: Optional[int] = None, ldb: Optional[int] = None, ldc: Optional[int] = None,
          a_kmajor: bool = False, b_kmajor: bool = False, Cin: Optional[torch.Tensor] = None,
          ldcin: Optional[int] = None, a_map=None, b_map=None, c_map=None, alpha: float = 1.0,
-         a_rows: Optional[int] = None, b_rows: Optional[int] = None, planes: bool = True):
+         a_rows: Optional[int] = None, b_rows: Optional[int] = None, planes: bool = True, rider: Optional[dict] = None):
     hip.require_gpu(A, "A")
     assert A.dtype == B.dtype, (A.dtype, B.dtype)
+    if rider is not None:
+        A2, B2, C2 = rider["A"], rider["B"], rider["C"]
+        hip.require_gpu(A2, "rider A")
+        assert A.dtype in H16 and C_.dtype == A.dtype and A2.dtype == A.dtype and B2.dtype == A.dtype and C2.dtype == A.dtype, \
+            "gemm(rider=): 16-bit operands and outputs of one type"
+        assert not a_kmajor and Cin is None and a_map is None and b_map is None and c_map is None and alpha == 1.0, \
+            "gemm(rider=): plain row-major-A problems only"
+        lda = lda if lda is not None else A.shape[-1]
+        ldb = ldb if ldb is not None else B.shape[-1]
+        ldc = ldc if ldc is not None else C_.shape[-1]
+        descs = [_GemmGroupDesc(ptr(A), ptr(B), ptr(C_), None, None, None,
+                                a_rows if a_rows is not None else A.numel() // lda, b_rows if b_rows is not None else B.numel() // ldb,
+                                M, N, K, lda, ldb, ldc, 0, 0, 0, 0),
+                 _GemmGroupDesc(ptr(A2), ptr(B2), ptr(C2), None, None, None, A2.numel() // A2.shape[-1], B2.numel() // B2.shape[-1],
+                                rider["M"], rider["N"], rider["K"], A2.shape[-1], B2.shape[-1], C2.shape[-1], 0, 0, 0, 0)]
+        _gemm_group(descs, 0, b_kmajor, A.dtype, A.device)
+        return
     lda = lda if lda is not None else A.shape[-1]
     ldb = ldb if ldb is not None else B.shape[-1]
     ldc = ldc if ldc is not None else C_.shape[-1]
@@ -299,10 +329,23 @@
 _DBIAS_RETIRED = []
 
 
-def gemm_qknorm(A, B, C_, scale, norm_out, groups, *, M, N, K, C2=None, c2_col0=0):
+def gemm_qknorm(A, B, C_, scale, norm_out, groups, *, M, N, K, C2=None, c2_col0=0, rider: Optional[dict] = None):
     hip.require_gpu(A, "A")
     assert A.dtype in H16 and B.dtype == A.dtype and C_.dtype == A.dtype and norm_out.dtype == torch.float32 and scale.dtype == torch.float32
     assert C2 is None or C2.dtype == A.dtype
+    if rider is not None:
+        def desc(A, B, C_, scale, norm_out, groups, M, N, K, C2=None, c2_col0=0):
+            hip.require_gpu(A, "A")
+            assert A.dtype in H16 and B.dtype == A.dtype and C_.dtype == A.dtype and norm_out.dtype == torch.float32 and scale.dtype == torch.float32
+            assert C2 is None or C2.dtype == A.dtype
+            return _GemmGroupDesc(ptr(A), ptr(B), ptr(C_), ptr(C2), ptr(scale), ptr(norm_out), A.numel() // A.shape[-1], B.numel() // B.shape[-1],
+                                  M, N, K, A.shape[-1], B.shape[-1], C_.shape[-1], C2.shape[-1] if C2 is not None else 0, int(c2_col0),
+                                  norm_out.shape[-1] if norm_out.dim() > 1 else 1, int(groups))
+        assert rider["A"].dtype == A.dtype, "gemm_qknorm(rider=): one operand type"
+        second = dict(rider)
+        second["C_"] = second.pop("C")
+        _gemm_group([desc(A, B, C_, scale, norm_out, groups, M, N, K, C2, c2_col0), desc(**second)], 1, False, A.dtype, A.device)
+        return
     call("omlm_gemm_qknorm", ptr(A), ptr(B), ptr(C_), ptr(C2), int(c2_col0), C2.shape[-1] if C2 is not None else 0, ptr(scale), ptr(norm_out),
          norm_out.shape[-1] if norm_out.dim() > 1 else 1, int(groups), A.numel() // A.shape[-1], B.numel() // B.shape[-1], M, N, K,
          A.shape[-1], B.shape[-1], C_.shape[-1], dcode(A.dtype), stream_ptr())
@@ -440,6 +483,12 @@
 
 def ffmid_bwd_workspace_floats(F, Fp) -> int:
     return int(hip.lib().omlm_ffmid_bwd_workspace_bytes(F, Fp)) // 4
+
+
+def ffmid_bwd_scratch_elems(M, Fp, dtype, p, have_drop_bits, have_gh) -> int:
+    nbytes = int(hip.lib().omlm_ffmid_bwd_scratch_bytes(int(M), int(Fp), int(bool(have_gh)), float(p), int(bool(have_drop_bits)), dcode(dtype)))
+    esz = torch.empty(0, dtype=dtype).element_size()
+    return (nbytes + esz - 1) // esz
 
 
 def ffmid_bwd(dh2, h1, convw, gamma, mean, rstd, du_tmp, dh1, dgamma, dconv, workspace, nseq, F, Fp, p, seed, seed_dev=None,
```

Result: no change. 1159 samples/s, median of 6 (+0.5%).
